# alexkeroro86/SampleNeRFRO

Measured on AMD Instinct MI355X. Metric: rays/sec (train step), higher is better.
Workload: dtype f16x3/fp32-acc

## Files before the change

### samplenerfro_amd/csrc/bkgd16.hip

```cpp
#include "mfma_ops.h"
#include "bkgd_layout.h"
#include "so3_layout.h"

namespace rnerf {

__device__ __forceinline__ void bkgd16_split2(float a, float b, uint32_t& hi, uint32_t& lo) { split2<true>(a, b, hi, lo); }
__device__ __forceinline__ void bkgd16_split8(const float (&w)[8], uint4& hi, uint4& lo) {
  uint32_t h[4], l[4];
#pragma unroll
  for (int p = 0; p < 4; ++p) bkgd16_split2(w[2 * p], w[2 * p + 1], h[p], l[p]);
  hi = make_uint4(h[0], h[1], h[2], h[3]); lo = make_uint4(l[0], l[1], l[2], l[3]);
}
template <int NS, bool FIRST, typename WF, typename LF, typename XF>
__device__ __forceinline__ void bkgd16_layer(f32x16 (&acc)[4], WF wload, LF live, bool half0, XF xop) {
  constexpr int DEPTH = 2;
  f32x2 w[DEPTH + 1][16];
  auto load = [&](int s, f32x2 (&dst)[16]) {
#pragma unroll
    for (int t = 0; t < 4; ++t)
#pragma unroll
      for (int j = 0; j < 8; ++j)
        if (live(s, j) != 0) dst[4 * t + (j >> 1)][j & 1] = wload(s, t, j);
  };
#pragma unroll
  for (int s = 0; s < DEPTH && s < NS; ++s) load(s, w[s]);
  f32x16 zero;
#pragma unroll
  for (int r = 0; r < 16; ++r) zero[r] = 0.f;
#pragma unroll
  for (int s = 0; s < NS; ++s) {
    if (s + DEPTH < NS) load(s + DEPTH, w[(s + DEPTH) % (DEPTH + 1)]);
    RNERF_PIN();
    uint4 bh, bl;
    xop(s, bh, bl);
#pragma unroll
    for (int t = 0; t < 4; ++t) {
      uint32_t hh[4], ll[4];
#pragma unroll
      for (int p = 0; p < 4; ++p) {
        const int l0 = live(s, 2 * p), l1 = live(s, 2 * p + 1);
        if (l0 == 0 && l1 == 0) { hh[p] = 0u; ll[p] = 0u; continue; }
        f32x2 q = w[s % (DEPTH + 1)][4 * t + p];
        if (l0 == 0) q[0] = 0.f;
        if (l1 == 0) q[1] = 0.f;
        q = q * 256.0f;
        if (l0 == 2) q[0] = half0 ? q[0] : 0.f;
        if (l1 == 2) q[1] = half0 ? q[1] : 0.f;
        bkgd16_split2(q[0], q[1], hh[p], ll[p]);
      }
      const uint4 ah = make_uint4(hh[0], hh[1], hh[2], hh[3]), al = make_uint4(ll[0], ll[1], ll[2], ll[3]);
      acc[t] = mfma16<true>(ah, bh, FIRST && s == 0 ? zero : acc[t]);
      acc[t] = mfma16<true>(ah, bl, acc[t]);
      acc[t] = mfma16<true>(al, bh, acc[t]);
    }
    RNERF_PIN();
  }
}
struct Bkgd16Lane {
  const float* p0;
  const float* prev;
  const float* dir;
  const float* sp;
  bool half0;
};
__device__ __forceinline__ Bkgd16Lane bkgd16_lane(const float* __restrict__ params, int m, int h) {
  return {params + m, params + m + 4 * 128 * h, params + m + 12 * 128 * h, params + m + 2 * 128 * h, h == 0};
}
template <bool BIAS>
__device__ __forceinline__ void bkgd16_prev_layer(f32x16 (&acc)[4], const f32x16 (&x)[4], const Bkgd16Lane& L, int koff, int boff) {
  bkgd16_layer<BIAS ? 9 : 8, true>(acc,
      [&](int s, int t, int j) { return s < 8 ? L.prev[koff + (16 * s + 8 * (j >> 2) + (j & 3)) * 128 + 32 * t] : L.p0[boff + 32 * t]; },
      [&](int s, int j) { return s < 8 ? 1 : (j == 0 ? 2 : 0); }, L.half0,
      [&](int s, uint4& bh, uint4& bl) {
    if (s < 8) {
      float xv[8];
#pragma unroll
      for (int j = 0; j < 8; ++j) xv[j] = x[s >> 1][8 * (s & 1) + j];
      bkgd16_split8(xv, bh, bl);
    } else {
      bh = make_uint4(L.half0 ? 0x3c00u : 0u, 0u, 0u, 0u);
      bl = make_uint4(0u, 0u, 0u, 0u);
    }
  });
}
template <bool FIRST>
__device__ __forceinline__ void bkgd16_dir_layer(f32x16 (&acc)[4], const float (&enc)[14], const Bkgd16Lane& L, int koff, int boff) {
  bkgd16_layer<2, FIRST>(acc,
      [&](int s, int t, int j) {
        const int q = 8 * s + j;
        return q < 12 ? L.dir[koff + (3 + q) * 128 + 32 * t] : (q == 12 ? L.sp[koff + 32 * t] : (q == 13 ? L.p0[koff + 128 + 32 * t] : L.p0[boff + 32 * t]));
      },
      [&](int s, int j) { const int q = 8 * s + j; return q < 13 ? 1 : (q < 15 ? 2 : 0); }, L.half0,
      [&](int s, uint4& bh, uint4& bl) {
    float xv[8];
#pragma unroll
    for (int j = 0; j < 8; ++j) xv[j] = 8 * s + j < 14 ? enc[8 * s + j] : (8 * s + j == 14 && L.half0 ? 1.0f : 0.f);
    bkgd16_split8(xv, bh, bl);
  });
}

template <bool TRAIN>
__global__ void __launch_bounds__(64) bkgd16_fwd_kernel(const float* __restrict__ params, const float* __restrict__ dirs, int dir_stride,
                                                        long long n, float pad_scale, float pad, float* __restrict__ out_rgb,
                                                        float* __restrict__ save) {
  const int lane = threadIdx.x & 63, m = lane & 31, h = lane >> 5;
  long long row = (long long)blockIdx.x * 32 + m;
  const bool ok = row < n;
  if (!ok) row = n - 1;
  const float v0 = dirs[row * dir_stride], v1 = dirs[row * dir_stride + 1], v2 = dirs[row * dir_stride + 2];
  float enc[14];
  const float phase = h ? 1.5707963705062866f : 0.0f;
#pragma unroll
  for (int q = 0; q < 12; ++q) {
    const int d = q / 3, c = q % 3;
    const float x = c == 0 ? v0 : (c == 1 ? v1 : v2);
    enc[q] = sinf(fadd(fmul(x, (float)(1 << d)), phase));
  }
  enc[12] = h ? v2 : v0;
  enc[13] = h ? 0.f : v1;
  auto save_x = [&](int k, const f32x16 (&xx)[4]) {
    if constexpr (TRAIN) {
      if (ok) {
        float* dst = save + (size_t)n * 28 + (size_t)(k - 1) * n * 128 + (size_t)row * 128;
#pragma unroll
        for (int t = 0; t < 4; ++t)
#pragma unroll
          for (int g = 0; g < 4; ++g)
            *(float4*)(dst + 32 * t + 8 * g + 4 * h) = make_float4(xx[t][4 * g], xx[t][4 * g + 1], xx[t][4 * g + 2], xx[t][4 * g + 3]);
      }
    }
  };
  if constexpr (TRAIN) {
    if (ok) {
#pragma unroll
      for (int q = 0; q < 14; ++q) { const int f = h ? dir_feature(q, 1) : dir_feature(q, 0); if (f >= 0) save[(size_t)row * 28 + f] = enc[q]; }
      if (h == 1) save[(size_t)row * 28 + 27] = 0.f;
    }
  }
  constexpr float INV = 1.0f / 256.0f;
  f32x16 acc[4], x[4];
  auto relu_to_x = [&]() {
#pragma unroll
    for (int t = 0; t < 4; ++t)
#pragma unroll
      for (int r = 0; r < 16; ++r) { const float y = acc[t][r] * INV; x[t][r] = y < 0.f ? 0.f : y; }
  };
  const Bkgd16Lane L = bkgd16_lane(params, m, h);
  bkgd16_dir_layer<true>(acc, enc, L, bkgd_koff(0), bkgd_boff(0));
  relu_to_x();
  save_x(1, x);
  bkgd16_prev_layer<true>(acc, x, L, bkgd_koff(1), bkgd_boff(1));
  relu_to_x();
  save_x(2, x);
  bkgd16_prev_layer<true>(acc, x, L, bkgd_koff(2), bkgd_boff(2));
  relu_to_x();
  save_x(3, x);
  bkgd16_prev_layer<false>(acc, x, L, bkgd_koff(3), 0);
  bkgd16_dir_layer<false>(acc, enc, L, bkgd_koff(3) + 128 * 128, bkgd_boff(3));
  relu_to_x();
  if constexpr (TRAIN) save_x(4, x);
  float o[3] = {0.f, 0.f, 0.f};
  const float* __restrict__ k4 = params + bkgd_koff(4);
#pragma unroll
  for (int t = 0; t < 4; ++t)
#pragma unroll
    for (int r = 0; r < 16; ++r) {
      const float v = x[t][r];
      const int f = 32 * t + (r & 3) + 8 * (r >> 2) + 4 * h;
      o[0] = fmaf(v, k4[f * 3 + 0], o[0]); o[1] = fmaf(v, k4[f * 3 + 1], o[1]); o[2] = fmaf(v, k4[f * 3 + 2], o[2]);
    }
#pragma unroll
  for (int c = 0; c < 3; ++c) {
    o[c] = o[c] + __shfl_xor(o[c], 32) + params[bkgd_boff(4) + c];
    o[c] = fsub(fmul(fdiv(1.0f, fadd(1.0f, expf(-o[c]))), pad_scale), pad);
  }
  if (ok && h == 0) {
    out_rgb[3 * row] = o[0]; out_rgb[3 * row + 1] = o[1]; out_rgb[3 * row + 2] = o[2];
    if constexpr (TRAIN) { float* so = save + (size_t)n * (28 + 4 * 128) + (size_t)row * 3; so[0] = o[0]; so[1] = o[1]; so[2] = o[2]; }
  }
}

static int launch_bkgd16_fwd(bool train, const float* params, const float* dirs, int dir_stride, long long n, float pad_scale, float pad, float* out_rgb,
                             float* save, hipStream_t st) {
  const dim3 grid((unsigned)((n + 31) / 32));
  if (train) hipLaunchKernelGGL(bkgd16_fwd_kernel<true>, grid, dim3(64), 0, st, params, dirs, dir_stride, n, pad_scale, pad, out_rgb, save);
  else hipLaunchKernelGGL(bkgd16_fwd_kernel<false>, grid, dim3(64), 0, st, params, dirs, dir_stride, n, pad_scale, pad, out_rgb, save);
  RNERF_CHECK_LAUNCH();
  return RNERF_OK;
}

template <bool FIRST>
__device__ __forceinline__ void so3_16_enc_layer(f32x16 (&acc)[4], const float (&enc)[30], const float* __restrict__ pe, const Bkgd16Lane& L, int koff, int boff) {
  bkgd16_layer<4, FIRST>(acc,
      [&](int s, int t, int j) { const int p = 8 * s + j; return p < 30 ? pe[koff + 2 * p * 128 + 32 * t] : L.p0[boff + 32 * t]; },
      [&](int s, int j) { const int p = 8 * s + j; return p < 30 ? 1 : (p == 30 ? 2 : 0); }, L.half0,
      [&](int s, uint4& bh, uint4& bl) {
    float xv[8];
#pragma unroll
    for (int j = 0; j < 8; ++j) { const int p = 8 * s + j; xv[j] = p < 30 ? enc[p < 30 ? p : 0] : ((p == 30 && L.half0) ? 1.0f : 0.f); }
    bkgd16_split8(xv, bh, bl);
  });
}

__global__ void __launch_bounds__(64) so3_16_fwd_train_kernel(const float* __restrict__ params, So3Window win, const float4* __restrict__ pts, long long n,
                                                              float* __restrict__ save) {
  const int lane = threadIdx.x & 63, m = lane & 31, h = lane >> 5;
  long long row = (long long)blockIdx.x * 32 + m;
  const bool ok = row < n;
  if (!ok) row = n - 1;
  const float4 pt = pts[row];
  float enc[30];
  so3_encode(pt.x, pt.y, pt.z, win, h, enc);
  if (ok) {
#pragma unroll
    for (int p = 0; p < 30; ++p) save[(size_t)row * 60 + 2 * p + h] = enc[p];
  }
  auto save_x = [&](int k, const f32x16 (&xx)[4]) {
    so3_store_mask(save, n, row, k, xx, h, ok);
    if (ok) {
      float* dst = save + (size_t)n * 60 + (size_t)(k - 1) * n * 128 + (size_t)row * 128;
#pragma unroll
      for (int t = 0; t < 4; ++t)
#pragma unroll
        for (int g = 0; g < 4; ++g)
          *(float4*)(dst + 32 * t + 8 * g + 4 * h) = make_float4(xx[t][4 * g], xx[t][4 * g + 1], xx[t][4 * g + 2], xx[t][4 * g + 3]);
    }
  };
  constexpr float INV = 1.0f / 256.0f;
  f32x16 acc[4], x[4];
  auto relu_to_x = [&]() {
#pragma unroll
    for (int t = 0; t < 4; ++t)
#pragma unroll
      for (int r = 0; r < 16; ++r) { const float y = acc[t][r] * INV; x[t][r] = y < 0.f ? 0.f : y; }
  };
  const Bkgd16Lane L = bkgd16_lane(params, m, h);
  const float* __restrict__ pe = params + m + 128 * h;
  so3_16_enc_layer<true>(acc, enc, pe, L, so3_koff(0), so3_boff(0));
  relu_to_x();
  save_x(1, x);
  bkgd16_prev_layer<true>(acc, x, L, so3_koff(1), so3_boff(1));
  relu_to_x();
  save_x(2, x);
  bkgd16_prev_layer<true>(acc, x, L, so3_koff(2), so3_boff(2));
  relu_to_x();
  save_x(3, x);
  bkgd16_prev_layer<false>(acc, x, L, so3_koff(3), 0);
  so3_16_enc_layer<false>(acc, enc, pe, L, so3_koff(3) + 128 * 128, so3_boff(3));
  relu_to_x();
  save_x(4, x);
  float o[3] = {0.f, 0.f, 0.f};
  const float* __restrict__ k4 = params + so3_koff(4);
#pragma unroll
  for (int t = 0; t < 4; ++t)
#pragma unroll
    for (int r = 0; r < 16; ++r) {
      const int f = 32 * t + (r & 3) + 8 * (r >> 2) + 4 * h;
      o[0] = fmaf(x[t][r], k4[f * 3 + 0], o[0]); o[1] = fmaf(x[t][r], k4[f * 3 + 1], o[1]); o[2] = fmaf(x[t][r], k4[f * 3 + 2], o[2]);
    }
#pragma unroll
  for (int c = 0; c < 3; ++c) o[c] = o[c] + __shfl_xor(o[c], 32) + params[so3_boff(4) + c];
  if (ok && h == 0) *(float4*)(save + (size_t)n * (60 + 4 * 128) + (size_t)row * 4) = make_float4(o[0], o[1], o[2], 0.f);
}

static int launch_so3_16_fwd_train(const float* params, So3Window win, const float* pts4, long long n, float* save, hipStream_t st) {
  hipLaunchKernelGGL(so3_16_fwd_train_kernel, dim3((unsigned)((n + 31) / 32)), dim3(64), 0, st, params, win, (const float4*)pts4, n, save);
  RNERF_CHECK_LAUNCH();
  return RNERF_OK;
}

}

using namespace rnerf;

extern "C" int rnerf_bkgd_forward(const float* params, const float* dirs, int32_t dir_stride, int64_t n, double rgb_padding,
                                  float* out_rgb, void* stream) {
  RNERF_CHECK_ARG(params && dirs && out_rgb, "rnerf_bkgd_forward: null pointer");
  RNERF_CHECK_ARG(dir_stride >= 3, "rnerf_bkgd_forward: dir_stride must be >= 3");
  RNERF_CHECK_ARG(n >= 1, "rnerf_bkgd_forward: n must be >= 1");
  return launch_bkgd16_fwd(false, params, dirs, dir_stride, (long long)n, (float)(1 + 2 * rgb_padding), (float)rgb_padding, out_rgb, nullptr, (hipStream_t)stream);
}

extern "C" int rnerf_bkgd_forward_train(const float* params, const float* dirs, int32_t dir_stride, int64_t n, double rgb_padding,
                                        float* out_rgb, void* save, void* stream) {
  RNERF_CHECK_ARG(params && dirs && out_rgb && save, "rnerf_bkgd_forward_train: null pointer");
  RNERF_CHECK_ARG(dir_stride >= 3 && n >= 1, "rnerf_bkgd_forward_train: need dir_stride >= 3 and n >= 1");
  return launch_bkgd16_fwd(true, params, dirs, dir_stride, (long long)n, (float)(1 + 2 * rgb_padding), (float)rgb_padding, out_rgb, (float*)save, (hipStream_t)stream);
}

extern "C" int rnerf_so3_forward_train(const float* so3_params, const float* window10, const float* pts4, int64_t n, void* save, void* stream) {
  RNERF_CHECK_ARG(so3_params && window10 && pts4 && save, "rnerf_so3_forward_train: null pointer");
  RNERF_CHECK_ARG(n >= 1, "rnerf_so3_forward_train: n must be >= 1");
  So3Window w;
  for (int i = 0; i < 10; ++i) w.w[i] = window10[i];
  return launch_so3_16_fwd_train(so3_params, w, pts4, (long long)n, (float*)save, (hipStream_t)stream);
}
```

### samplenerfro_amd/csrc/mlp.hip

```cpp
#include "common.h"
#include "nerfmlp_layout.h"
#include "mfma_ops.h"

#include <stdlib.h>
#include <type_traits>
#include <vector>
#include <stdio.h>

namespace rnerf {


#define GLOBAL_AS __attribute__((address_space(1)))
#define LDS_AS __attribute__((address_space(3)))

struct MfmaLayer { int dense, ks, nt, kind; };
__host__ __device__ constexpr MfmaLayer mfma_layer(int l) {
  constexpr MfmaLayer t[10] = {{0, 4, 8, 0},  {1, 16, 8, 1}, {2, 16, 8, 1}, {3, 16, 8, 1}, {4, 16, 8, 1},
                               {5, 20, 8, 2}, {6, 16, 8, 1}, {7, 16, 8, 1}, {9, 16, 8, 1}, {10, 18, 4, 3}};
  return t[l];
}
__host__ __device__ constexpr int layer_blocks_before(int l) {
  int o = 0;
  for (int i = 0; i < l; ++i) o += mfma_layer(i).ks * mfma_layer(i).nt;
  return o;
// ... 1397 lines not shown
    const int t = b / NP, part = b % NP;
    int slot0, slot1;
    const uint4* base;
    WgTrDma d;
    if (t < KT) {
      x_slots(sg, t, slot0, slot1);
      base = saved + (part ? sv_lo0(R) : 0);
      d.tstride = (unsigned)(SAVE_SLOTS * 64 * sizeof(uint4));
    } else {
      d_slots(sg, t - KT, slot0, slot1);
      base = dy + (part ? dy_plane_uint4(R, 1) : 0);
      d.tstride = (unsigned)(DY_SLOTS * 64 * sizeof(uint4));
    }
    static_assert(sv_addr(1, 0, 0, 0) == dy_addr(1, 0, 0, 0) && sv_addr(0, 0, 1, 1) == dy_addr(0, 0, 1, 1), "one lane-offset formula for both tensors");
    d.sbase = (const char*)(base + sv_addr(__builtin_amdgcn_readfirstlane(slot0), 0, 0, 0));
    d.voff = (unsigned)((sv_addr(a ? __builtin_amdgcn_readfirstlane(slot1 - slot0) : 0, 0, r, h)) * sizeof(uint4));
    d.hstride = 0;
    return d;
  }
  static __device__ __forceinline__ const char* step_src(const WgTrDma& d, size_t t32, int sc) {
    return d.sbase + t32 * d.tstride + (sc & 1) * (32 * sizeof(uint4));
  }
  template <int KT, int NT> struct Frags {
    const char* ring;
    __device__ __forceinline__ Frags(const char* ring0, int lane) : ring(ring0 + wgtr_lane_off(lane)) {}
    __device__ __forceinline__ void read_a(int t, const half8& sc8, half8& h, half8& l) const {
      const char* p = ring + t * NP * 1024;
      h = tr_read8(p) * sc8;
      if constexpr (LO) l = tr_read8(p + 1024) * sc8;
    }
    __device__ __forceinline__ void read_b(int nt, half8& h, half8& l) const {
      const char* p = ring + (KT + nt) * NP * 1024;
      h = tr_read8(p);
      if constexpr (LO) l = tr_read8(p + 1024);
    }
  };
};

__device__ __forceinline__ int2v tr_read8b(const char* p) {
  typedef __attribute__((address_space(3))) int2v lds_int2;
  return __builtin_amdgcn_ds_read_tr8_b64_v2i32((lds_int2*)p);
}
struct Lo8Planes {
  static constexpr bool LO = true;
  static constexpr int NPLANES = 2;
  static constexpr int NBUF = 4;
  static constexpr int nblk(int KT, int NT) { return KT + NT + (KT + 1) / 2 + (NT + 1) / 2; }
  static constexpr int lds_bytes() { return NBUF * wgtr_step_bytes(nblk(10, 8)); }
  template <int KT, int NT>
  static __device__ __forceinline__ WgTrDma dma(int b, int lane, const uint4* __restrict__ saved, const uint4* __restrict__ dy, long long R, const WgTrSegs& sg) {
    constexpr int NHI = KT + NT, NLX = (KT + 1) / 2;
    WgTrDma d;
    if (b < NHI) {
      const int r = lane >> 2, a = (lane >> 1) & 1, h = lane & 1;
      int s0, s1;
      const bool is_x = b < KT;
      if (is_x) x_slots(sg, b, s0, s1); else d_slots(sg, b - KT, s0, s1);
      d.sbase = (const char*)((is_x ? saved : dy) + sv_addr(__builtin_amdgcn_readfirstlane(s0), 0, 0, 0));
      d.voff = (unsigned)((sv_addr(a ? __builtin_amdgcn_readfirstlane(s1 - s0) : 0, 0, r, h)) * sizeof(uint4));
      d.tstride = (unsigned)((is_x ? SAVE_SLOTS : DY_SLOTS) * 64 * sizeof(uint4));
      d.hstride = (unsigned)(32 * sizeof(uint4));
      return d;
    }
    const int lb = b - NHI;
    const bool is_x = lb < NLX;
    const int t0 = 2 * (is_x ? lb : lb - NLX) + (lane >> 5);
    const int r = (lane & 31) >> 1, a = lane & 1;
    int s0, s1;
    if (is_x) x_slots(sg, t0 < KT ? t0 : KT - 1, s0, s1); else d_slots(sg, t0 < NT ? t0 : NT - 1, s0, s1);
    d.sbase = is_x ? (const char*)(saved + sv_lo0(R)) : (const char*)(dy + dy_plane_uint4(R, 1));
    d.voff = (unsigned)(((a ? s1 : s0) * 32 + r) * 16);
    d.tstride = (unsigned)((is_x ? SAVE_SLOTS : DY_SLOTS) * 32 * 16);
    d.hstride = 16u * 16u;
    return d;
  }
  static __device__ __forceinline__ const char* step_src(const WgTrDma& d, size_t t32, int sc) {
    return d.sbase + t32 * d.tstride + (sc & 1) * d.hstride;
  }
  template <int KT, int NT> struct Frags {
    static constexpr int LOX = (KT + NT) * 1024, LOD = LOX + (KT + 1) / 2 * 1024;
    const char *ring, *ring8;
    __device__ __forceinline__ Frags(const char* ring0, int lane)
        : ring(ring0 + wgtr_lane_off(lane)), ring8(ring0 + (unsigned)((8 * (lane >> 5) + ((lane & 15) >> 1)) * 32 + ((lane >> 4) & 1) * 16 + (lane & 1) * 8)) {}
    __device__ __forceinline__ void read_a(int t, const half8& sc8, half8& h, half8& l) const {
      h = tr_read8(ring + t * 1024) * sc8;
      l = lo8_decode(tr_read8b(ring8 + LOX + t * 512), LO8_SCALE_X) * sc8;
    }
    __device__ __forceinline__ void read_b(int nt, half8& h, half8& l) const {
      h = tr_read8(ring + (KT + nt) * 1024);
      l = lo8_decode(tr_read8b(ring8 + LOD + nt * 512), LO8_SCALE_D);
    }
  };
};

template <class Planes, int KT, int NT>
__device__ __forceinline__ void wgrad_body_tr(const uint4* __restrict__ saved, const uint4* __restrict__ dy, long long R, float* __restrict__ pg,
                                               float* __restrict__ pbias, const WgTrSegs sg, int g, int G, char* smem) {
  using SH = WgTrShape<KT, NT>;
  constexpr int TK = SH::TK, TN = SH::TN;
  constexpr int NBLK = Planes::nblk(KT, NT), NDMA = (NBLK + 7) / 8, STEP_BYTES = wgtr_step_bytes(NBLK);
  constexpr int WGTR_NBUF = Planes::NBUF, AHEAD = WGTR_NBUF - 1;
  static_assert((WGTR_NBUF & (WGTR_NBUF - 1)) == 0, "ring slots are addressed with a mask");
  const int tid = threadIdx.x, lane = tid & 63;
  const int wave = __builtin_amdgcn_readfirstlane(tid >> 6);
  const int wk = wave / SH::WN, wn = wave % SH::WN;
  const bool active = wave < SH::WK * SH::WN;
  const float* __restrict__ rs = (const float*)(dy + dy_plane_uint4(R, Planes::NPLANES));
  const float mref = rs[R];
  const float inv_mref = mref > 0.f ? 1.0f / mref : 0.f;
  WgTrDma blk[NDMA];
  unsigned lds_blk[NDMA];
#pragma unroll
  for (int i = 0; i < NDMA; ++i) {
    int b = wave + 8 * i;
    b = b < NBLK ? b : NBLK - 1;
    blk[i] = Planes::template dma<KT, NT>(b, lane, saved, dy, R, sg);
    lds_blk[i] = (unsigned)b * 1024u;
  }
  const float* rs_src = rs + 4 * (lane & 3);
  const long long n_t32 = R / 32;
  const int my_tiles = g < n_t32 ? (int)((n_t32 - 1 - g) / G) + 1 : 0;
  const int n_steps = 2 * my_tiles;
  auto issue = [&](int s) {
    const int sc = s < n_steps ? s : n_steps - 1;
    const size_t t32 = (size_t)g + (size_t)(sc >> 1) * G;
    const unsigned ring = (unsigned)(s & (WGTR_NBUF - 1)) * STEP_BYTES;
#pragma unroll
    for (int i = 0; i < NDMA; ++i)
      glds16_nt_s(Planes::step_src(blk[i], t32, sc), blk[i].voff, __builtin_amdgcn_readfirstlane(ring + lds_blk[i]));
    if (wave == 0) glds16_nt((const char*)(rs_src + t32 * 32 + (sc & 1) * 16), __builtin_amdgcn_readfirstlane(ring + NBLK * 1024u));
  };
  const f32x16 zero = {0, 0, 0, 0, 0, 0, 0, 0, 0, 0, 0, 0, 0, 0, 0, 0};
  f32x16 acc[TK][TN], acce = zero;
  float accb = 0.f;
#pragma unroll
  for (int i = 0; i < TK; ++i)
#pragma unroll
    for (int j = 0; j < TN; ++j) acc[i][j] = zero;
  if (n_steps > 0) {
#pragma unroll
    for (int s = 0; s < AHEAD; ++s) issue(s);
    const int kh = lane >> 5;
    for (int s = 0; s < n_steps; ++s) {
      if (wave == 0) wait_vmcnt<(AHEAD - 1) * (NDMA + 1)>(); else
      wait_vmcnt<(AHEAD - 1) * NDMA>();
      __syncthreads();
      issue(s + AHEAD);
      if (active) {
        const char* ring0 = smem + (s & (WGTR_NBUF - 1)) * STEP_BYTES;
        const typename Planes::template Frags<KT, NT> frags(ring0, lane);
        const float4 s0 = *(const float4*)(ring0 + NBLK * 1024 + kh * 32), s1 = *(const float4*)(ring0 + NBLK * 1024 + kh * 32 + 16);
        const half8 sc8 = {(_Float16)(s0.x * inv_mref), (_Float16)(s0.y * inv_mref), (_Float16)(s0.z * inv_mref), (_Float16)(s0.w * inv_mref),
                           (_Float16)(s1.x * inv_mref), (_Float16)(s1.y * inv_mref), (_Float16)(s1.z * inv_mref), (_Float16)(s1.w * inv_mref)};
        half8 beh, bel;
        if constexpr (SH::EXTRA) frags.read_b(NT - 1, beh, bel);
        static_assert(SH::WK >= TN, "bias owners");
        auto read_a = [&](int i, half8& h, half8& l) { frags.read_a(wk * TK + i, sc8, h, l); };
        auto read_b = [&](int j, half8& h, half8& l) { frags.read_b(wn * TN + j, h, l); };
        auto dot8 = [&](const half8& x, float c) -> float {
#pragma unroll
          for (int k = 0; k < 4; ++k) c = __builtin_amdgcn_fdot2(half2v{sc8[2 * k], sc8[2 * k + 1]}, half2v{x[2 * k], x[2 * k + 1]}, c, false);
          return c;
        };
        auto bias_row = [&](int j, const half8& h, const half8& l) {
          if (wk == j) {
            accb = dot8(h, accb);
            if constexpr (Planes::LO) accb = dot8(l, accb);
          }
        };
        half8 ae_h, ae_l;
        if constexpr (TK > TN) {
          half8 bh[TN], bl[TN];
#pragma unroll
          for (int j = 0; j < TN; ++j) read_b(j, bh[j], bl[j]);
          half8 an_h, an_l;
          read_a(0, an_h, an_l);
#pragma unroll
          for (int i = 0; i < TK; ++i) {
            const half8 ah = an_h, al = an_l;
            if (i + 1 < TK) read_a(i + 1, an_h, an_l);
#pragma unroll
            for (int j = 0; j < TN; ++j) acc[i][j] = mfma_h8(ah, bh[j], acc[i][j]);
            if constexpr (Planes::LO) {
#pragma unroll
              for (int j = 0; j < TN; ++j) acc[i][j] = mfma_h8(ah, bl[j], acc[i][j]);
#pragma unroll
              for (int j = 0; j < TN; ++j) acc[i][j] = mfma_h8(al, bh[j], acc[i][j]);
            }
          }
#pragma unroll
          for (int j = 0; j < TN; ++j) bias_row(j, bh[j], bl[j]);
        } else {
          constexpr int NCH = WGTR_NCH < TN ? WGTR_NCH : TN;
          static_assert(TN % NCH == 0, "n-tile chunks");
          half8 ah[TK], al[TK];
#pragma unroll
          for (int i = 0; i < TK; ++i) read_a(i, ah[i], al[i]);
#pragma unroll
          for (int c = 0; c < TN / NCH; ++c) {
            half8 bh[NCH], bl[NCH];
#pragma unroll
            for (int jj = 0; jj < NCH; ++jj) read_b(c * NCH + jj, bh[jj], bl[jj]);
#pragma unroll
            for (int i = 0; i < TK; ++i)
#pragma unroll
              for (int jj = 0; jj < NCH; ++jj) acc[i][c * NCH + jj] = mfma_h8(ah[i], bh[jj], acc[i][c * NCH + jj]);
            if constexpr (Planes::LO) {
#pragma unroll
              for (int i = 0; i < TK; ++i)
#pragma unroll
                for (int jj = 0; jj < NCH; ++jj) acc[i][c * NCH + jj] = mfma_h8(ah[i], bl[jj], acc[i][c * NCH + jj]);
#pragma unroll
              for (int i = 0; i < TK; ++i)
#pragma unroll
                for (int jj = 0; jj < NCH; ++jj) acc[i][c * NCH + jj] = mfma_h8(al[i], bh[jj], acc[i][c * NCH + jj]);
            }
#pragma unroll
            for (int jj = 0; jj < NCH; ++jj) bias_row(c * NCH + jj, bh[jj], bl[jj]);
          }
          if constexpr (SH::EXTRA) { ae_h = wn ? ah[1] : ah[0]; if constexpr (Planes::LO) ae_l = wn ? al[1] : al[0]; }
        }
        if constexpr (SH::EXTRA) {
          static_assert(!SH::EXTRA || TK <= TN, "the extra tile reads the resident A fragments");
          acce = mfma_h8(ae_h, beh, acce);
          if constexpr (Planes::LO) {
            acce = mfma_h8(ae_h, bel, acce);
            acce = mfma_h8(ae_l, beh, acce);
          }
        }
      }
    }
    wait_vmcnt<0>();
  }
  constexpr size_t ldn = (size_t)NT * 32;
  const int m = lane & 31, h = lane >> 5;
  if (active) {
#pragma unroll
    for (int i = 0; i < TK; ++i)
#pragma unroll
      for (int j = 0; j < TN; ++j)
#pragma unroll
        for (int r = 0; r < 16; ++r) {
          const int row = (r & 3) + 8 * (r >> 2) + 4 * h;
          pg[(size_t)((wk * TK + i) * 32 + row) * ldn + (wn * TN + j) * 32 + m] = acc[i][j][r];
        }
    if constexpr (SH::EXTRA) {
#pragma unroll
      for (int r = 0; r < 16; ++r) {
        const int row = (r & 3) + 8 * (r >> 2) + 4 * h;
        pg[(size_t)((wk * TK + wn) * 32 + row) * ldn + (NT - 1) * 32 + m] = acce[r];
      }
    }
    const float bsum = accb + __shfl_xor(accb, 32);
    if (wk < TN && h == 0) pbias[(wn * TN + wk) * 32 + m] = bsum;
  }
}

constexpr int WGRAD_VGPRS = 112;
template <class Planes>
__global__ void __launch_bounds__(512) __attribute__((amdgpu_num_vgpr(WGRAD_VGPRS)))
nerfmlp_wgrad_tr_kernel(const uint4* __restrict__ saved, const uint4* __restrict__ dy, long long R, float* __restrict__ workspace, const WgradTable tab,
                        long long* __restrict__ trace) {
  extern __shared__ __attribute__((aligned(16))) char smem[];
  if (trace && threadIdx.x == 0) trace[2 * blockIdx.x] = (long long)__builtin_amdgcn_s_memrealtime();
  int j = 0;
  while ((int)blockIdx.x >= tab.wg0[j + 1]) ++j;
  const WgradJob job = tab.job[j];
  const int g = blockIdx.x - tab.wg0[j], G = tab.wg0[j + 1] - tab.wg0[j];
  const int KT = job.KT, NT = job.NT;
  float* pg = workspace + tab.poff[j] + (size_t)g * (size_t)KT * 32 * NT * 32;
  float* pb = workspace + tab.pboff[j] + (size_t)g * NT * 32;
  const WgTrSegs sg = {tab.qx[j], job.KTa, tab.qx2[j], tab.qd[j], job.NTa, tab.KSd[j], tab.qd2[j], tab.KSd2[j]};
#define RNERF_WGRAD_CASE(KT_, NT_)                                                                                                  \
  if (KT == (KT_) && NT == (NT_)) {                                                                                                 \
    wgrad_body_tr<Planes, KT_, NT_>(saved, dy, R, pg, pb, sg, g, G, smem);                                                          \
    if (trace && threadIdx.x == 0) trace[2 * blockIdx.x + 1] = (long long)__builtin_amdgcn_s_memrealtime();                         \
    return;                                                                                                                         \
  }
  RNERF_WGRAD_CASE(8, 8) RNERF_WGRAD_CASE(2, 8) RNERF_WGRAD_CASE(10, 8) RNERF_WGRAD_CASE(8, 9) RNERF_WGRAD_CASE(9, 4) RNERF_WGRAD_CASE(4, 1)
#undef RNERF_WGRAD_CASE
  __builtin_trap();
}

template <bool X_F16>
__global__ void __launch_bounds__(512)
nerfmlp_wgrad_kernel(const uint4* __restrict__ saved, const uint4* __restrict__ dy, long long R, long long total_rows, int n_chunks,
                      float* __restrict__ workspace, const WgradTable tab) {
  extern __shared__ __attribute__((aligned(16))) char smem[];
  int j = 0;
  while ((int)blockIdx.x >= tab.wg0[j + 1]) ++j;
  const int qx = tab.qx[j], KSx = tab.KSx[j], qd = tab.qd[j], KSd = tab.KSd[j];
  const int g = blockIdx.x - tab.wg0[j], G = tab.wg0[j + 1] - tab.wg0[j];
  const int KT = KSx >> 1, NT = (KSd + 1) >> 1;
  float* pg = workspace + tab.poff[j] + (size_t)g * (size_t)KT * 32 * NT * 32;
  float* pb = workspace + tab.pboff[j] + (size_t)g * NT * 32;
#define RNERF_WGRAD_CASE(KT_, KSD_)                                                                                                 \
  if (KSx == 2 * (KT_) && KSd == (KSD_)) { wgrad_body<X_F16, KT_, KSD_>(saved, dy, R, total_rows, n_chunks, pg, pb, qx, qd, g, G, smem); return; }
  RNERF_WGRAD_CASE(8, 16) RNERF_WGRAD_CASE(2, 16) RNERF_WGRAD_CASE(8, 1) RNERF_WGRAD_CASE(8, 8) RNERF_WGRAD_CASE(1, 8) RNERF_WGRAD_CASE(4, 1)
#undef RNERF_WGRAD_CASE
  __builtin_trap();
}

__global__ void __launch_bounds__(256) wgrad_reduce_kernel(const float* __restrict__ workspace, const WgradTable tab, float* __restrict__ grads,
                                                           const float* __restrict__ out_scale) {
  const float osc = out_scale ? *out_scale : 1.0f;
  const int jb = blockIdx.y;
  const WgradJob job = tab.job[jb];
  const int n_wg = tab.wg0[jb + 1] - tab.wg0[jb];
  const float* __restrict__ partial = workspace + tab.poff[jb];
  const float* __restrict__ partial_bias = workspace + tab.pboff[jb];
  const int ldn = job.NT * 32, rows = job.KT * 32;
  const int e = blockIdx.x * blockDim.x + threadIdx.x;
  auto out_feature = [&](int J, int& dense) -> int {
    int nt = J >> 5;
    const int c = J & 31, a = c >> 4, hh = (c >> 3) & 1, j = c & 7;
    const bool segb = nt >= job.NTa;
    const int dkind = segb ? job.dkind2 : job.dkind;
    dense = segb ? job.dense2 : job.dense;
    if (segb) nt -= job.NTa;
    if (dkind == 0) { const int n = prev_feature(2 * nt + a, hh, j); return n < nerf_dense(dense).out ? n : -1; }
    if (a != 0 || hh != 0 || nt != 0) return -1;
    if (dkind == 1) return j == 0 ? 0 : -1;
    return (j >= 1 && j <= 3) ? j - 1 : -1;
  };
  auto sum_over = [&](const float* __restrict__ p, size_t stride) -> float {
    float s0 = 0.f, s1 = 0.f, s2 = 0.f, s3 = 0.f;
    int g = 0;
    for (; g + 4 <= n_wg; g += 4) { s0 += p[(size_t)g * stride]; s1 += p[(size_t)(g + 1) * stride]; s2 += p[(size_t)(g + 2) * stride]; s3 += p[(size_t)(g + 3) * stride]; }
    for (; g < n_wg; ++g) s0 += p[(size_t)g * stride];
    return (s0 + s1) + (s2 + s3);
  };
  if (e < rows * ldn) {
    const int I = e / ldn, J = e % ldn;
    int kt = I >> 5;
    const int c = I & 31, a = c >> 4, hh = (c >> 3) & 1, j = c & 7;
    const bool segb = kt >= job.KTa;
    const int xkind = segb ? job.xkind2 : job.xkind, row_off = segb ? job.row_off2 : job.row_off;
    if (segb) kt -= job.KTa;
    const int s = 2 * kt + a;
    int fin = xkind == 1 ? prev_feature(s, hh, j) : (xkind == 0 ? pe_feature(8 * s + j, hh) : view_feature(8 * s + j, hh));
    int dense;
    const int fout = out_feature(J, dense);
    if (fin >= 0 && fout >= 0) {
      fin += row_off;
      if (fin < nerf_dense(dense).in) grads[nerf_koff(dense) + fin * nerf_dense(dense).out + fout] = sum_over(partial + e, (size_t)rows * ldn) * osc;
    }
  }
  if (job.write_bias && e < ldn) {
    int dense;
    const int fout = out_feature(e, dense);
    if (fout >= 0 && (e >> 5) < job.NTa) grads[nerf_boff(dense) + fout] = sum_over(partial_bias + e, (size_t)ldn) * osc;
    if (job.bias_sigma && e == 0) grads[nerf_boff(8)] = sum_over(partial_bias, (size_t)ldn) * osc;
  }
}

template <int NP>
__global__ void __launch_bounds__(64) nerfmlp_input_grad_kernel(const float* __restrict__ params, const uint4* __restrict__ dy, long long R,
                                                                const float4* __restrict__ rows_pd, const float4* __restrict__ rows_dr,
                                                                const int* __restrict__ node_of_sample, int B, long long total_rows,
                                                                float4* __restrict__ d_pos, float4* __restrict__ d_dir) {
  const int lane = threadIdx.x & 63, m = lane & 31, h = lane >> 5;
  long long row = (long long)blockIdx.x * 32 + m;
  const bool ok = row < total_rows;
  if (!ok) row = total_rows - 1;
  const f32x16 zero = {0, 0, 0, 0, 0, 0, 0, 0, 0, 0, 0, 0, 0, 0, 0, 0};
  f32x16 dpe[2] = {zero, zero}, dve = zero;
  auto slot_vals = [&](int q, float (&vals)[8]) {
    const uint4 hi = dy[dy_addr(q, row >> 5, (int)(row & 31), h)];
    const uint32_t hw[4] = {hi.x, hi.y, hi.z, hi.w};
#pragma unroll
    for (int p = 0; p < 4; ++p) unpack2<true>(hw[p], vals[2 * p], vals[2 * p + 1]);
    if constexpr (NP == 2) {
      const uint4 lo = dy[dy_plane_uint4(R, 1) + dy_addr(q, row >> 5, (int)(row & 31), h)];
      const uint32_t lw[4] = {lo.x, lo.y, lo.z, lo.w};
#pragma unroll
      for (int p = 0; p < 4; ++p) { float a, b; unpack2<true>(lw[p], a, b); vals[2 * p] += a; vals[2 * p + 1] += b; }
    }
    if constexpr (NP == 3) {
      const uint2 lo = ((const uint2*)(dy + dy_plane_uint4(R, 1)))[dy_addr(q, row >> 5, (int)(row & 31), h)];
      const half8 lv = lo8_decode(int2v{(int)lo.x, (int)lo.y}, LO8_SCALE_D);
#pragma unroll
      for (int j = 0; j < 8; ++j) vals[j] += (float)lv[j];
    }
  };
  auto gemm_T = [&](const float* __restrict__ kern, int out_dim, int row0, int fin, int slot0, int nslots, f32x16* acc, int ntile) {
    const float* __restrict__ kr[2];
    bool live[2];
#pragma unroll
    for (int t2 = 0; t2 < 2; ++t2) {
      const int f = 32 * t2 + m;
      live[t2] = f < fin;
      kr[t2] = kern + (size_t)(row0 + (f < fin ? f : fin - 1)) * out_dim + 4 * h;
    }
    float4 wc[2][2], wn[2][2];
    float vc[8], vn[8];
    auto fetch = [&](int s, float4 (&w)[2][2], float (&vals)[8]) {
#pragma unroll
      for (int t2 = 0; t2 < 2; ++t2)
        if (t2 < ntile) { w[t2][0] = *(const float4*)(kr[t2] + 16 * s); w[t2][1] = *(const float4*)(kr[t2] + 16 * s + 8); }
      slot_vals(slot0 + s, vals);
    };
    fetch(0, wc, vc);
#pragma unroll 1
    for (int s = 0; s < nslots; ++s) {
      if (s + 1 < nslots) fetch(s + 1, wn, vn);
      RNERF_PIN();
#pragma unroll
      for (int j = 0; j < 8; ++j) {
#pragma unroll
        for (int t2 = 0; t2 < 2; ++t2) {
          if (t2 < ntile) {
            const float4 q = wc[t2][j >> 2];
            const float w = (j & 3) == 0 ? q.x : ((j & 3) == 1 ? q.y : ((j & 3) == 2 ? q.z : q.w));
            acc[t2] = __builtin_amdgcn_mfma_f32_32x32x2f32(live[t2] ? w : 0.f, vc[j], acc[t2], 0, 0, 0);
          }
        }
      }
      RNERF_PIN();
#pragma unroll
      for (int t2 = 0; t2 < 2; ++t2) { wc[t2][0] = wn[t2][0]; wc[t2][1] = wn[t2][1]; }
#pragma unroll
      for (int j = 0; j < 8; ++j) vc[j] = vn[j];
    }
  };
  gemm_T(params + nerf_koff(0), 256, 0, 63, 0, 16, dpe, 2);
  gemm_T(params + nerf_koff(5), 256, 256, 63, 16 * 5, 16, dpe, 2);
  gemm_T(params + nerf_koff(10), 128, 256, 27, DY_L9, 8, &dve, 1);
  size_t rec = (size_t)row;
  if (node_of_sample) { const long long sidx = row / B; rec = (size_t)node_of_sample[sidx] * B + (size_t)(row - sidx * B); }
  const float4 pd = rows_pd[rec], dr = rows_dr[rec];
  const float pc[3] = {pd.x, pd.y, pd.z}, dcv[3] = {dr.x, dr.y, dr.z};
  const float HALF_PI = 1.5707963705062866f;
  float gp3[3] = {0.f, 0.f, 0.f}, gd3[3] = {0.f, 0.f, 0.f};
#pragma unroll
  for (int t2 = 0; t2 < 2; ++t2)
#pragma unroll
    for (int r = 0; r < 16; ++r) {
      const int f = 32 * t2 + (r & 3) + 8 * (r >> 2) + 4 * h;
      if (f < 3) gp3[f] += dpe[t2][r];
      else if (f < 63) {
        const int q = (f - 3) % 30, is_cos = (f - 3) / 30, d = q / 3, c = q % 3;
        const float xb = fmul(pc[c], (float)(1 << d));
        gp3[c] = fmaf(dpe[t2][r], (float)(1 << d) * pe_cos(is_cos ? fadd(xb, HALF_PI) : xb), gp3[c]);
      }
    }
#pragma unroll
  for (int r = 0; r < 16; ++r) {
    const int f = (r & 3) + 8 * (r >> 2) + 4 * h;
    if (f < 3) gd3[f] += dve[r];
    else if (f < 27) {
      const int q = (f - 3) % 12, is_cos = (f - 3) / 12, d = q / 3, c = q % 3;
      const float xb = fmul(dcv[c], (float)(1 << d));
      gd3[c] = fmaf(dve[r], (float)(1 << d) * pe_cos(is_cos ? fadd(xb, HALF_PI) : xb), gd3[c]);
    }
  }
  const float* __restrict__ rs = (const float*)(dy + dy_plane_uint4(R, NP == 3 ? 2 : NP));
  const float sc = rs[row];
#pragma unroll
  for (int c = 0; c < 3; ++c) { gp3[c] = (gp3[c] + __shfl_xor(gp3[c], 32)) * sc; gd3[c] = (gd3[c] + __shfl_xor(gd3[c], 32)) * sc; }
  if (ok && h == 0) { d_pos[row] = make_float4(gp3[0], gp3[1], gp3[2], 0.f); d_dir[row] = make_float4(gd3[0], gd3[1], gd3[2], 0.f); }
}

}

namespace rnerf {
int launch_fwd_f32(const void* packed, const float* rows_pd, const float* rows_dr, const int32_t* node_of_sample, int32_t B, long long total_rows,
                   float* out_raw, hipStream_t st);
}

using namespace rnerf;

constexpr size_t kF8Fallback = (Prec<RNERF_PREC_F16F8>::PACKED_BYTES + 255) & ~(size_t)255;

constexpr size_t kX3Bytes = (Prec<RNERF_PREC_F16X3>::PACKED_BYTES + 255) & ~(size_t)255;
constexpr size_t kSafeBytes = Prec<RNERF_PREC_BF16X3>::PACKED_BYTES;
constexpr size_t kF16Bytes = (Prec<RNERF_PREC_F16>::PACKED_BYTES + 255) & ~(size_t)255;
static size_t safe_stream_offset(int precision) {
  switch (precision) {
    case RNERF_PREC_F16X3:
    case RNERF_PREC_F16X2: return kX3Bytes;
    case RNERF_PREC_F16F8: return kF8Fallback + kX3Bytes;
    case RNERF_PREC_F16: return kF16Bytes;
    default: return 0;
  }
}

#define RNERF_TRY_(expr) do { int rc_ = (expr); if (rc_ != RNERF_OK) return rc_; } while (0)

static bool prec_ok(int p) {
  return p == RNERF_PREC_F32 || p == RNERF_PREC_F16X3 || p == RNERF_PREC_BF16X3 || p == RNERF_PREC_F16 || p == RNERF_PREC_BF16 || p == RNERF_PREC_F16X2 || p == RNERF_PREC_F16F8;
}

extern "C" size_t rnerf_nerfmlp_packed_bytes(int precision) {
  switch (precision) {
    case RNERF_PREC_F32: return (size_t)RNERF_NERFMLP_PARAMS * sizeof(float);
    case RNERF_PREC_F16X3:
    case RNERF_PREC_F16X2: return kX3Bytes + kSafeBytes;
    case RNERF_PREC_F16F8: return kF8Fallback + kX3Bytes + kSafeBytes;
    case RNERF_PREC_BF16X3: return Prec<RNERF_PREC_BF16X3>::PACKED_BYTES;
    case RNERF_PREC_F16: return kF16Bytes + kSafeBytes;
    case RNERF_PREC_BF16: return Prec<RNERF_PREC_BF16>::PACKED_BYTES;
    default: set_error("rnerf_nerfmlp_packed_bytes: unsupported precision %d", precision); return 0;
  }
}

namespace rnerf {
void* nerfmlp_dgrad_scale_ref(int backward, void* dy, int64_t rows);
static int pack_flag_regions(int precision, void* packed, void** out) {
  auto at = [&](size_t off) { return (void*)((char*)packed + off + AUX_FLAG * sizeof(float)); };
  switch (precision) {
    case RNERF_PREC_F16X3:
    case RNERF_PREC_F16X2: out[0] = at(Prec<RNERF_PREC_F16X3>::STREAM_BYTES); return 1;
    case RNERF_PREC_F16F8: out[0] = at(Prec<RNERF_PREC_F16F8>::STREAM_BYTES); out[1] = at(kF8Fallback + Prec<RNERF_PREC_F16X3>::STREAM_BYTES); return 2;
    case RNERF_PREC_F16: out[0] = at(Prec<RNERF_PREC_F16>::STREAM_BYTES); return 1;
    default: return 0;
  }
}
struct FlagRegions { float4* p[12]; };
__global__ void __launch_bounds__(64) zero_flags_kernel(FlagRegions r, int n) {
  if ((int)threadIdx.x < n) *r.p[threadIdx.x] = make_float4(0.f, 0.f, 0.f, 0.f);
}
int nerfmlp_step_zero(int precision, void* const* packed, int count, int backward, void* const* dy, const int64_t* dy_rows, int dy_count, hipStream_t st) {
  FlagRegions r;
  int n = 0;
  for (int i = 0; i < count && i < 2; ++i) { void* o[2]; const int k = pack_flag_regions(precision, packed[i], o); for (int q = 0; q < k; ++q) r.p[n++] = (float4*)o[q]; }
  for (int i = 0; i < dy_count && i < 4; ++i) { void* f = nerfmlp_dgrad_scale_ref(backward, dy[i], dy_rows[i]); if (f) r.p[n++] = (float4*)f; }
  if (n == 0) return RNERF_OK;
  hipLaunchKernelGGL(zero_flags_kernel, dim3(1), dim3(64), 0, st, r, n);
  RNERF_CHECK_LAUNCH();
  return RNERF_OK;
}

int nerfmlp_pack_impl(const float* params, int precision, void* packed, bool zero_flags, hipStream_t st, bool with_safe) {
  const int threads = kTotalBlocks * 64, block = 256, grid = (threads + block - 1) / block;
  if (zero_flags) {
    void* o[2];
    const int k = pack_flag_regions(precision, packed, o);
    for (int q = 0; q < k; ++q) RNERF_CHECK_HIP(hipMemsetAsync(o[q], 0, 4 * sizeof(float), st));
  }
  switch (precision) {
    case RNERF_PREC_F32:
      RNERF_CHECK_HIP(hipMemcpyAsync(packed, params, (size_t)RNERF_NERFMLP_PARAMS * sizeof(float), hipMemcpyDeviceToDevice, st));
      return RNERF_OK;
    case RNERF_PREC_F16X3:
    case RNERF_PREC_F16X2: hipLaunchKernelGGL(nerfmlp_pack_kernel<RNERF_PREC_F16X3>, dim3(grid), dim3(block), 0, st, params, (char*)packed); break;
    case RNERF_PREC_F16F8:
      hipLaunchKernelGGL(nerfmlp_pack_kernel<RNERF_PREC_F16F8>, dim3(grid), dim3(block), 0, st, params, (char*)packed);
      hipLaunchKernelGGL(nerfmlp_pack_kernel<RNERF_PREC_F16X3>, dim3(grid), dim3(block), 0, st, params, (char*)packed + kF8Fallback);
      break;
    case RNERF_PREC_F16: hipLaunchKernelGGL(nerfmlp_pack_kernel<RNERF_PREC_F16>, dim3(grid), dim3(block), 0, st, params, (char*)packed); break;
    case RNERF_PREC_BF16X3: hipLaunchKernelGGL(nerfmlp_pack_kernel<RNERF_PREC_BF16X3>, dim3(grid), dim3(block), 0, st, params, (char*)packed); break;
    default: hipLaunchKernelGGL(nerfmlp_pack_kernel<RNERF_PREC_BF16>, dim3(grid), dim3(block), 0, st, params, (char*)packed); break;
  }
  if (with_safe && safe_stream_offset(precision) != 0)
    hipLaunchKernelGGL(nerfmlp_pack_kernel<RNERF_PREC_BF16X3>, dim3(grid), dim3(block), 0, st, params, (char*)packed + safe_stream_offset(precision));
  RNERF_CHECK_LAUNCH();
  return RNERF_OK;
}
}

extern "C" int rnerf_nerfmlp_pack(const float* params, int precision, void* packed, void* stream) {
  RNERF_CHECK_ARG(params && packed, "rnerf_nerfmlp_pack: null pointer");
  RNERF_CHECK_ARG(prec_ok(precision), "rnerf_nerfmlp_pack: unsupported precision %d", precision);
  RNERF_CHECK_ARG(((uintptr_t)packed & 15) == 0, "rnerf_nerfmlp_pack: packed must be 16-byte aligned");
  return nerfmlp_pack_impl(params, precision, packed, true, (hipStream_t)stream, true);
}

constexpr size_t SAVE_QUEUE_BYTES = 8192;
static size_t save_payload_bytes(long long padded, bool with_lo) {
  return (size_t)(SAVE_TOTAL + (with_lo ? SAVE_SLOTS : 0)) * (size_t)padded * 2 * sizeof(uint4);
}

template <int PREC, int MODE = 0, int TRAIN = 0>
static int launch_fwd_mode(const void* packed, const float* rows_pd, const float* rows_dr, const int32_t* node_of_sample, int32_t B,
                           long long total_rows, float* out_raw, hipStream_t st, void* save = nullptr, int max_wg = 0, const float* gate = nullptr,
                           int gate_skip_if = 0) {
  using PP = Prec<PREC>;
  const int n_tiles = (int)((total_rows + 255) / 256);
  int dev = 0, cus = 0;
  RNERF_CHECK_HIP(hipGetDevice(&dev));
  RNERF_CHECK_HIP(hipDeviceGetAttribute(&cus, hipDeviceAttributeMultiprocessorCount, dev));
  const int lim = (max_wg > 0 && max_wg < cus) ? max_wg : cus;
  if constexpr (MODE == 0 && (PREC == RNERF_PREC_F16X3 || PREC == RNERF_PREC_F16F8)) {
    static const bool half_ok = [] { const char* e = RNERF_ENV("RNERF_FWD_HALF_TILES"); return !(e && e[0] == '0'); }();
    if (half_ok && 2 * n_tiles <= lim) {
      const size_t lds1 = 2 * (size_t)PP::SLAB;
      static DeviceOnce attr1_set;
      if (attr1_set.need()) {
        RNERF_CHECK_HIP(hipFuncSetAttribute((const void*)nerfmlp_fwd_kernel<PREC, 0, TRAIN, true>, hipFuncAttributeMaxDynamicSharedMemorySize, (int)lds1));
        attr1_set.set();
      }
      hipLaunchKernelGGL((nerfmlp_fwd_kernel<PREC, 0, TRAIN, true>), dim3(2 * n_tiles), dim3(256), lds1, st, (const char*)packed, (const float4*)rows_pd,
                         (const float4*)rows_dr, node_of_sample, B, total_rows, 2 * n_tiles, (float4*)out_raw, (uint4*)save, (long long)n_tiles * 256,
                         (int*)nullptr, gate, gate_skip_if);
      RNERF_CHECK_LAUNCH();
      return RNERF_OK;
    }
  }
  const int grid = n_tiles < lim ? n_tiles : lim;
  const size_t lds = 2 * (size_t)PP::SLAB + 4 * 32768;
  static DeviceOnce attr_set;
  if (attr_set.need()) {
    RNERF_CHECK_HIP(hipFuncSetAttribute((const void*)nerfmlp_fwd_kernel<PREC, MODE, TRAIN>, hipFuncAttributeMaxDynamicSharedMemorySize, (int)lds));
    attr_set.set();
  }
  int* tileq = nullptr;
  if (TRAIN != 0 && grid < cus && grid < n_tiles) {
    tileq = (int*)((char*)save + save_payload_bytes((long long)n_tiles * 256, TRAIN >= 2));
    RNERF_CHECK_HIP(hipMemsetAsync(tileq, 0, sizeof(int), st));
  }
  hipLaunchKernelGGL((nerfmlp_fwd_kernel<PREC, MODE, TRAIN>), dim3(grid), dim3(256), lds, st, (const char*)packed, (const float4*)rows_pd,
                     (const float4*)rows_dr, node_of_sample, B, total_rows, n_tiles, (float4*)out_raw, (uint4*)save,
                     (long long)n_tiles * 256, tileq, gate, gate_skip_if);
  RNERF_CHECK_LAUNCH();
  return RNERF_OK;
}

template <int PREC>
static int launch_fwd(const void* packed, const float* rows_pd, const float* rows_dr, const int32_t* node_of_sample, int32_t B,
                      long long total_rows, float* out_raw, hipStream_t st, int max_wg, const float* gate = nullptr, int gate_skip_if = 0) {
  return launch_fwd_mode<PREC>(packed, rows_pd, rows_dr, node_of_sample, B, total_rows, out_raw, st, nullptr, max_wg, gate, gate_skip_if);
}

extern "C" int rnerf_nerfmlp_forward(const void* packed, int precision, const float* rows_pd, const float* rows_dr,
                                     const int32_t* node_of_sample, int32_t S, int32_t B, float* out_raw, int32_t max_workgroups,
                                     void* stream) {
  RNERF_CHECK_ARG(packed && rows_pd && rows_dr && out_raw, "rnerf_nerfmlp_forward: null pointer");
  RNERF_CHECK_ARG(max_workgroups >= 0, "rnerf_nerfmlp_forward: max_workgroups must be >= 0");
  RNERF_CHECK_ARG(prec_ok(precision), "rnerf_nerfmlp_forward: unsupported precision %d", precision);
  RNERF_CHECK_ARG(S >= 1 && B >= 1, "rnerf_nerfmlp_forward: need S >= 1 and B >= 1");
  RNERF_CHECK_ARG((((uintptr_t)packed | (uintptr_t)rows_pd | (uintptr_t)rows_dr | (uintptr_t)out_raw) & 15) == 0,
                  "rnerf_nerfmlp_forward: buffers must be 16-byte aligned");
  const long long total = (long long)S * B;
  hipStream_t st = (hipStream_t)stream;
  switch (precision) {
    case RNERF_PREC_F32: return launch_fwd_f32(packed, rows_pd, rows_dr, node_of_sample, B, total, out_raw, st);
    case RNERF_PREC_F16X3:
      RNERF_TRY_(launch_fwd<RNERF_PREC_F16X3>(packed, rows_pd, rows_dr, node_of_sample, B, total, out_raw, st, max_workgroups));
      return launch_fwd_mode<RNERF_PREC_BF16X3, 512>((const char*)packed + safe_stream_offset(precision), rows_pd, rows_dr, node_of_sample, B, total, out_raw, st, nullptr, max_workgroups);
    case RNERF_PREC_F16X2:
      RNERF_TRY_(launch_fwd<RNERF_PREC_F16X2>(packed, rows_pd, rows_dr, node_of_sample, B, total, out_raw, st, max_workgroups));
      return launch_fwd_mode<RNERF_PREC_BF16X3, 512>((const char*)packed + safe_stream_offset(precision), rows_pd, rows_dr, node_of_sample, B, total, out_raw, st, nullptr, max_workgroups);
    case RNERF_PREC_F16F8: {
      const float* flag = (const float*)((const char*)packed + Prec<RNERF_PREC_F16F8>::STREAM_BYTES) + AUX_FLAG;
      RNERF_TRY_(launch_fwd<RNERF_PREC_F16F8>(packed, rows_pd, rows_dr, node_of_sample, B, total, out_raw, st, max_workgroups, flag, 1));
      RNERF_TRY_(launch_fwd<RNERF_PREC_F16X3>((const char*)packed + kF8Fallback, rows_pd, rows_dr, node_of_sample, B, total, out_raw, st, max_workgroups, flag, 0));
      return launch_fwd_mode<RNERF_PREC_BF16X3, 512>((const char*)packed + safe_stream_offset(precision), rows_pd, rows_dr, node_of_sample, B, total, out_raw, st, nullptr, max_workgroups);
    }
    case RNERF_PREC_BF16X3: return launch_fwd<RNERF_PREC_BF16X3>(packed, rows_pd, rows_dr, node_of_sample, B, total, out_raw, st, max_workgroups);
    case RNERF_PREC_F16:
      RNERF_TRY_(launch_fwd<RNERF_PREC_F16>(packed, rows_pd, rows_dr, node_of_sample, B, total, out_raw, st, max_workgroups));
      return launch_fwd_mode<RNERF_PREC_BF16X3, 512>((const char*)packed + safe_stream_offset(precision), rows_pd, rows_dr, node_of_sample, B, total, out_raw, st, nullptr, max_workgroups);
    default: return launch_fwd<RNERF_PREC_BF16>(packed, rows_pd, rows_dr, node_of_sample, B, total, out_raw, st, max_workgroups);
  }
}

static bool bwd_ok(int b) { return b == RNERF_BWD_BF16 || b == RNERF_BWD_F16 || b == RNERF_BWD_F16X2 || b == RNERF_BWD_F16X3_LO8; }
static bool bwd_two_planes(int b) { return b == RNERF_BWD_F16X2 || b == RNERF_BWD_F16X3_LO8; }
static bool train_combo_ok(int precision, int backward) {
  return precision == RNERF_PREC_F16X3 || (precision == RNERF_PREC_F16 && !bwd_two_planes(backward)) ||
         (precision == RNERF_PREC_BF16X3 && backward == RNERF_BWD_BF16);
}
static size_t train_stream_bytes(int precision) {
  return precision == RNERF_PREC_F16 ? Prec<RNERF_PREC_F16>::STREAM_BYTES : (precision == RNERF_PREC_BF16X3 ? Prec<RNERF_PREC_BF16X3>::STREAM_BYTES : Prec<RNERF_PREC_F16X3>::STREAM_BYTES);
}

extern "C" size_t rnerf_nerfmlp_save_bytes(int64_t rows, int backward) {
  const int64_t padded = (rows + 255) / 256 * 256;
  return save_payload_bytes(padded, bwd_two_planes(backward)) + SAVE_QUEUE_BYTES;
}

extern "C" int rnerf_nerfmlp_forward_train(const void* packed, int precision, const float* rows_pd, const float* rows_dr,
                                           const int32_t* node_of_sample, int32_t S, int32_t B, float* out_raw, void* save,
                                           int backward, int32_t max_workgroups, void* stream) {
  RNERF_CHECK_ARG(packed && rows_pd && rows_dr && out_raw && save, "rnerf_nerfmlp_forward_train: null pointer");
  RNERF_CHECK_ARG(max_workgroups >= 0, "rnerf_nerfmlp_forward_train: max_workgroups must be >= 0");
  RNERF_CHECK_ARG(bwd_ok(backward), "rnerf_nerfmlp_forward_train: unknown backward mode %d", backward);
  RNERF_CHECK_ARG(train_combo_ok(precision, backward),
                  "rnerf_nerfmlp_forward_train: the training forward is built for precision f16x3, f16 with the single-plane backward modes, and bf16x3 with backward bf16");
  RNERF_CHECK_ARG(S >= 1 && B >= 1, "rnerf_nerfmlp_forward_train: need S >= 1 and B >= 1");
  RNERF_CHECK_ARG((((uintptr_t)packed | (uintptr_t)rows_pd | (uintptr_t)rows_dr | (uintptr_t)out_raw | (uintptr_t)save) & 15) == 0,
                  "rnerf_nerfmlp_forward_train: buffers must be 16-byte aligned");
  const long long total = (long long)S * B;
  hipStream_t st = (hipStream_t)stream;
  if (backward == RNERF_BWD_F16X2) return launch_fwd_mode<RNERF_PREC_F16X3, 0, 2>(packed, rows_pd, rows_dr, node_of_sample, B, total, out_raw, st, save, max_workgroups);
  if (backward == RNERF_BWD_F16X3_LO8) return launch_fwd_mode<RNERF_PREC_F16X3, 0, 3>(packed, rows_pd, rows_dr, node_of_sample, B, total, out_raw, st, save, max_workgroups);
  if (precision == RNERF_PREC_BF16X3) return launch_fwd_mode<RNERF_PREC_BF16X3, 0, 1>(packed, rows_pd, rows_dr, node_of_sample, B, total, out_raw, st, save, max_workgroups);
  if (precision == RNERF_PREC_F16) return launch_fwd_mode<RNERF_PREC_F16, 0, 1>(packed, rows_pd, rows_dr, node_of_sample, B, total, out_raw, st, save, max_workgroups);
  return launch_fwd_mode<RNERF_PREC_F16X3, 0, 1>(packed, rows_pd, rows_dr, node_of_sample, B, total, out_raw, st, save, max_workgroups);
}

extern "C" size_t rnerf_nerfmlp_bwd_packed_bytes(void) { return (size_t)kBwdBlocks * 2 * 1024; }
extern "C" size_t rnerf_nerfmlp_dy_bytes(int64_t rows, int backward) {
  const int64_t padded = (rows + 255) / 256 * 256;
  const int np = bwd_two_planes(backward) ? 2 : 1;
  return dy_plane_uint4(padded, np) * sizeof(uint4) + (backward == RNERF_BWD_BF16 ? 0 : ((size_t)padded + 4) * sizeof(float));
}

extern "C" int rnerf_nerfmlp_pack_bwd(const float* params, int backward, void* packed_bwd, void* stream) {
  RNERF_CHECK_ARG(params && packed_bwd, "rnerf_nerfmlp_pack_bwd: null pointer");
  RNERF_CHECK_ARG(bwd_ok(backward), "rnerf_nerfmlp_pack_bwd: unknown backward mode %d", backward);
  const int threads = kBwdBlocks * 64;
  if (backward == RNERF_BWD_BF16)
    hipLaunchKernelGGL(nerfmlp_pack_bwd_kernel<RNERF_PREC_BF16X3>, dim3((threads + 255) / 256), dim3(256), 0, (hipStream_t)stream, params, (char*)packed_bwd);
  else
    hipLaunchKernelGGL(nerfmlp_pack_bwd_kernel<RNERF_PREC_F16X3>, dim3((threads + 255) / 256), dim3(256), 0, (hipStream_t)stream, params, (char*)packed_bwd);
  RNERF_CHECK_LAUNCH();
  return RNERF_OK;
}

void* rnerf::nerfmlp_dgrad_scale_ref(int backward, void* dy, int64_t rows) {
  const long long R = (rows + 255) / 256 * 256;
  if (bwd_two_planes(backward)) return (char*)dy + dy_plane_uint4(R, Bwd<RNERF_BWD_F16X2>::NP) * sizeof(uint4) + (size_t)R * sizeof(float);
  if (backward == RNERF_BWD_F16) return (char*)dy + dy_plane_uint4(R, Bwd<RNERF_BWD_F16>::NP) * sizeof(uint4) + (size_t)R * sizeof(float);
  return nullptr;
}

template <int BWD>
static int launch_dgrad(const void* packed_bwd, const float* fwd_aux, const void* save, const float* d_raw, int64_t rows, void* dy, hipStream_t st,
                        bool zero_ref = true, bool allow_half = true) {
  using PB = Prec<Bwd<BWD>::PREC>;
  const int n_tiles = (int)((rows + 255) / 256);
  int dev = 0, cus = 0;
  RNERF_CHECK_HIP(hipGetDevice(&dev));
  RNERF_CHECK_HIP(hipDeviceGetAttribute(&cus, hipDeviceAttributeMultiprocessorCount, dev));
  const int grid = n_tiles < cus ? n_tiles : cus;
  const size_t lds = 2 * (size_t)PB::SLAB + 4 * 32768;
  static DeviceOnce attr_set;
  if (attr_set.need()) {
    RNERF_CHECK_HIP(hipFuncSetAttribute((const void*)nerfmlp_dgrad_kernel<BWD>, hipFuncAttributeMaxDynamicSharedMemorySize, (int)lds));
    attr_set.set();
  }
  const long long R = (long long)n_tiles * 256;
  if (Bwd<BWD>::F16 && zero_ref) RNERF_CHECK_HIP(hipMemsetAsync(nerfmlp_dgrad_scale_ref(BWD == kBwdF16OnePass ? RNERF_BWD_F16 : BWD, dy, rows), 0, 4 * sizeof(float), st));
  if constexpr (BWD == RNERF_BWD_F16X2 || BWD == RNERF_BWD_F16 || BWD == kBwdF16OnePass || BWD == RNERF_BWD_F16X3_LO8) {
    static const int half_lim = [] { const char* e = RNERF_ENV("RNERF_DGRAD_HALF_TILES"); return e ? atoi(e) : -1; }();
    if (allow_half && half_lim != 0 && 2 * n_tiles <= (half_lim > 1 ? half_lim : cus)) {
      const size_t lds1 = 2 * (size_t)PB::SLAB;
      static DeviceOnce attr1_set;
      if (attr1_set.need()) {
        RNERF_CHECK_HIP(hipFuncSetAttribute((const void*)nerfmlp_dgrad_kernel<BWD, true>, hipFuncAttributeMaxDynamicSharedMemorySize, (int)lds1));
        attr1_set.set();
      }
      hipLaunchKernelGGL((nerfmlp_dgrad_kernel<BWD, true>), dim3(2 * n_tiles), dim3(256), lds1, st, (const char*)packed_bwd, fwd_aux, (const uint4*)save, R,
                         (const float4*)d_raw, (long long)rows, 2 * n_tiles, (uint4*)dy);
      RNERF_CHECK_LAUNCH();
      return RNERF_OK;
    }
  }
  hipLaunchKernelGGL(nerfmlp_dgrad_kernel<BWD>, dim3(grid), dim3(256), lds, st, (const char*)packed_bwd, fwd_aux, (const uint4*)save, R,
                     (const float4*)d_raw, (long long)rows, n_tiles, (uint4*)dy);
  RNERF_CHECK_LAUNCH();
  return RNERF_OK;
}

namespace rnerf {
int nerfmlp_dgrad_impl(const void* packed_bwd, const void* packed_fwd, int fwd_precision, int backward, const void* save, const float* d_raw, int64_t rows,
                       void* dy, bool zero_ref, bool allow_half, hipStream_t st) {
  RNERF_CHECK_ARG(packed_bwd && packed_fwd && save && d_raw && dy, "rnerf_nerfmlp_dgrad: null pointer");
  RNERF_CHECK_ARG(train_combo_ok(fwd_precision, backward), "rnerf_nerfmlp_dgrad: forward precision must be f16x3 (f16 with a single-plane backward mode; bf16x3 with backward bf16)");
  RNERF_CHECK_ARG(bwd_ok(backward), "rnerf_nerfmlp_dgrad: unknown backward mode %d", backward);
  RNERF_CHECK_ARG(rows >= 1, "rnerf_nerfmlp_dgrad: rows must be >= 1");
  const float* fwd_aux = (const float*)((const char*)packed_fwd + train_stream_bytes(fwd_precision));
  if (backward == RNERF_BWD_F16X2) return launch_dgrad<RNERF_BWD_F16X2>(packed_bwd, fwd_aux, save, d_raw, rows, dy, st, zero_ref, allow_half);
  if (backward == RNERF_BWD_F16X3_LO8) return launch_dgrad<RNERF_BWD_F16X3_LO8>(packed_bwd, fwd_aux, save, d_raw, rows, dy, st, zero_ref, allow_half);
  if (backward == RNERF_BWD_F16 && fwd_precision == RNERF_PREC_F16) return launch_dgrad<kBwdF16OnePass>(packed_bwd, fwd_aux, save, d_raw, rows, dy, st, zero_ref, allow_half);
  if (backward == RNERF_BWD_F16) return launch_dgrad<RNERF_BWD_F16>(packed_bwd, fwd_aux, save, d_raw, rows, dy, st, zero_ref, allow_half);
  return launch_dgrad<RNERF_BWD_BF16>(packed_bwd, fwd_aux, save, d_raw, rows, dy, st, zero_ref, allow_half);
}
}

extern "C" int rnerf_nerfmlp_dgrad(const void* packed_bwd, const void* packed_fwd, int fwd_precision, int backward, const void* save,
                                   const float* d_raw, int64_t rows, void* dy, void* stream) {
  return nerfmlp_dgrad_impl(packed_bwd, packed_fwd, fwd_precision, backward, save, d_raw, rows, dy, true, true, (hipStream_t)stream);
}

struct WgradPlan { int qx, KSx, qd, KSd; WgradJob job; int qx2, qd2, KSd2; };
static constexpr WgradJob job1(int dense, int xkind, int row_off, int dkind, int KT, int NT, int wb, int bias_sigma = 0) {
  return WgradJob{dense, xkind, row_off, dkind, KT, NT, wb, KT, 0, 0, NT, 0, 0, bias_sigma};
}
static const WgradPlan kWgradPlan[15] = {
    {SAVE_PE, 4, 0, 16, job1(0, 0, 0, 0, 2, 8, 1), 0, 0, 0},
    {SAVE_L1 + 0, 16, 16, 16, job1(1, 1, 0, 0, 8, 8, 1), 0, 0, 0},   {SAVE_L1 + 16, 16, 32, 16, job1(2, 1, 0, 0, 8, 8, 1), 0, 0, 0},
    {SAVE_L1 + 32, 16, 48, 16, job1(3, 1, 0, 0, 8, 8, 1), 0, 0, 0},  {SAVE_L1 + 48, 16, 64, 16, job1(4, 1, 0, 0, 8, 8, 1), 0, 0, 0},
    {SAVE_L1 + 64, 16, 80, 16, job1(5, 1, 0, 0, 8, 8, 1), 0, 0, 0},  {SAVE_PE, 4, 80, 16, job1(5, 0, 256, 0, 2, 8, 0), 0, 0, 0},
    {SAVE_L1 + 80, 16, 96, 16, job1(6, 1, 0, 0, 8, 8, 1), 0, 0, 0},  {SAVE_L1 + 96, 16, 112, 16, job1(7, 1, 0, 0, 8, 8, 1), 0, 0, 0},
    {SAVE_L1 + 112, 16, 128, 16, job1(9, 1, 0, 0, 8, 8, 1), 0, 0, 0}, {SAVE_L1 + 112, 16, DY_HEADS, 1, job1(8, 1, 0, 1, 8, 1, 1), 0, 0, 0},
    {SAVE_L1 + 128, 16, DY_L9, 8, job1(10, 1, 0, 0, 8, 4, 1), 0, 0, 0}, {SAVE_VIEW, 2, DY_L9, 8, job1(10, 2, 256, 0, 1, 4, 0), 0, 0, 0},
    {SAVE_RGBIN, 8, DY_HEADS, 1, job1(11, 1, 0, 2, 4, 1, 1), 0, 0, 0},
    {0, 0, 0, 0, job1(0, 0, 0, 0, 0, 0, 0), 0, 0, 0}};
static const WgradPlan kWgradPlanTr[12] = {
    {SAVE_PE, 4, 0, 16, job1(0, 0, 0, 0, 2, 8, 1), 0, 0, 0},
    {SAVE_L1 + 0, 16, 16, 16, job1(1, 1, 0, 0, 8, 8, 1), 0, 0, 0},   {SAVE_L1 + 16, 16, 32, 16, job1(2, 1, 0, 0, 8, 8, 1), 0, 0, 0},
    {SAVE_L1 + 32, 16, 48, 16, job1(3, 1, 0, 0, 8, 8, 1), 0, 0, 0},  {SAVE_L1 + 48, 16, 64, 16, job1(4, 1, 0, 0, 8, 8, 1), 0, 0, 0},
    {SAVE_L1 + 64, 20, 80, 16, WgradJob{5, 1, 0, 0, 10, 8, 1,  8,  0,  256,  8, 0, 0, 0}, SAVE_PE, 0, 0},
    {SAVE_L1 + 80, 16, 96, 16, job1(6, 1, 0, 0, 8, 8, 1), 0, 0, 0},  {SAVE_L1 + 96, 16, 112, 16, job1(7, 1, 0, 0, 8, 8, 1), 0, 0, 0},
    {SAVE_L1 + 112, 16, 128, 16, WgradJob{9, 1, 0, 0, 8, 9, 1, 8, 0, 0,  8,  8,  1, 0}, 0, DY_HEADS, 1},
    {SAVE_L1 + 128, 18, DY_L9, 8, WgradJob{10, 1, 0, 0, 9, 4, 1,  8,  2,  256, 4, 0, 0, 0}, SAVE_VIEW, 0, 0},
    {SAVE_RGBIN, 8, DY_HEADS, 1, job1(11, 1, 0, 2, 4, 1, 1,  1), 0, 0, 0},
    {0, 0, 0, 0, job1(0, 0, 0, 0, 0, 0, 0), 0, 0, 0}};

static size_t build_wgrad_table(int cus, WgradTable& t, bool legacy, int mult = 0) {
  const WgradPlan* plan = legacy ? kWgradPlan : kWgradPlanTr;
  int n = 0;
  double cost[16], total = 0;
  for (; plan[n].KSx != 0; ++n) {
    const WgradJob& jb = plan[n].job;
    cost[n] = legacy ? 2.0 * jb.KT * jb.NT + 2 * (jb.KT + jb.NT) + 16 : jb.KT + jb.NT + 1;
    total += cost[n];
  }
  t.n = n;
  const int budget = (mult > 0 ? mult : (legacy ? 4 : 2)) * cus;
  size_t off = 0;
  int wg = 0;
  for (int i = 0; i < n; ++i) {
    const WgradPlan& p = plan[i];
    int share = (int)(budget * cost[i] / total + 0.5);
    if (share < 8) share = 8;
    t.qx[i] = p.qx; t.KSx[i] = p.KSx; t.qd[i] = p.qd; t.KSd[i] = p.KSd; t.job[i] = p.job;
    t.qx2[i] = p.qx2; t.qd2[i] = p.qd2; t.KSd2[i] = p.KSd2;
    t.wg0[i] = wg; wg += share;
    t.poff[i] = (long long)off; off += (size_t)share * p.job.KT * 32 * p.job.NT * 32;
    t.pboff[i] = (long long)off; off += (size_t)share * p.job.NT * 32;
  }
  t.wg0[n] = wg;
  return off;
}

static int device_cus() {
  int dev = 0, cus = 256;
  if (hipGetDevice(&dev) == hipSuccess) hipDeviceGetAttribute(&cus, hipDeviceAttributeMultiprocessorCount, dev);
  return cus;
}

constexpr long long kWgradSmallRows = 24576;
struct WgradTables { WgradTable legacy, tr, tr_small; size_t partial_floats; int max_wgs; };
static const WgradTables& wgrad_tables() {
  static const WgradTables tables = [] {
    WgradTables w;
    const size_t a = build_wgrad_table(device_cus(), w.legacy, true), b = build_wgrad_table(device_cus(), w.tr, false);
    const size_t s = build_wgrad_table(device_cus(), w.tr_small, false, 1);
    w.partial_floats = a > b ? a : b;
    if (s > w.partial_floats) w.partial_floats = s;
    w.max_wgs = w.legacy.wg0[w.legacy.n] > w.tr.wg0[w.tr.n] ? w.legacy.wg0[w.legacy.n] : w.tr.wg0[w.tr.n];
    if (w.tr_small.wg0[w.tr_small.n] > w.max_wgs) w.max_wgs = w.tr_small.wg0[w.tr_small.n];
    return w;
  }();
  return tables;
}

extern "C" size_t rnerf_nerfmlp_wgrad_workspace_bytes(void) {
  const WgradTables& w = wgrad_tables();
  return w.partial_floats * sizeof(float) + (size_t)w.max_wgs * 2 * sizeof(long long);
}

template <class Planes> struct WgradTrHost {
  static hipError_t allow_lds() {
    return hipFuncSetAttribute((const void*)nerfmlp_wgrad_tr_kernel<Planes>, hipFuncAttributeMaxDynamicSharedMemorySize, Planes::lds_bytes());
  }
  static const float* launch(const WgradTable& tab, hipStream_t st, const void* save, const void* dy, long long R, void* workspace, long long* trace) {
    hipLaunchKernelGGL(nerfmlp_wgrad_tr_kernel<Planes>, dim3(tab.wg0[tab.n]), dim3(512), Planes::lds_bytes(), st, (const uint4*)save, (const uint4*)dy, R,
                       (float*)workspace, tab, trace);
    return (const float*)((const uint4*)dy + dy_plane_uint4(R, Planes::NPLANES)) + R;
  }
};

extern "C" int rnerf_nerfmlp_wgrad(int fwd_precision, int backward, const void* save, const void* dy, int64_t rows, float* grads, void* workspace,
                                   void* stream) {
  RNERF_CHECK_ARG(save && dy && grads && workspace, "rnerf_nerfmlp_wgrad: null pointer");
  RNERF_CHECK_ARG(train_combo_ok(fwd_precision, backward), "rnerf_nerfmlp_wgrad: forward precision must be f16x3 (f16 with a single-plane backward mode; bf16x3 with backward bf16)");
  RNERF_CHECK_ARG(bwd_ok(backward), "rnerf_nerfmlp_wgrad: unknown backward mode %d", backward);
  RNERF_CHECK_ARG(rows >= 1, "rnerf_nerfmlp_wgrad: rows must be >= 1");
  const WgradTables& w = wgrad_tables();
  static DeviceOnce ready;
  if (ready.need()) {
    RNERF_CHECK_HIP(hipFuncSetAttribute((const void*)nerfmlp_wgrad_kernel<true>, hipFuncAttributeMaxDynamicSharedMemorySize, 131072));
    RNERF_CHECK_HIP(hipFuncSetAttribute((const void*)nerfmlp_wgrad_kernel<false>, hipFuncAttributeMaxDynamicSharedMemorySize, 131072));
    RNERF_CHECK_HIP(WgradTrHost<F16Planes<1>>::allow_lds());
    RNERF_CHECK_HIP(WgradTrHost<F16Planes<2>>::allow_lds());
    RNERF_CHECK_HIP(WgradTrHost<Lo8Planes>::allow_lds());
    ready.set();
  }
  const long long R = (rows + 255) / 256 * 256;
  hipStream_t st = (hipStream_t)stream;
  const float* out_scale = nullptr;
  static const bool tracing = RNERF_ENV("RNERF_WGRAD_TRACE") != nullptr;
  long long* trace = tracing ? (long long*)((char*)workspace + w.partial_floats * sizeof(float)) : nullptr;
  const WgradTable& tab = backward == RNERF_BWD_BF16 ? w.legacy : (rows <= kWgradSmallRows ? w.tr_small : w.tr);
  if (backward == RNERF_BWD_BF16) {
    const int n_chunks = (int)((rows + 127) / 128);
    if (fwd_precision == RNERF_PREC_BF16X3)
      hipLaunchKernelGGL(nerfmlp_wgrad_kernel<false>, dim3(tab.wg0[tab.n]), dim3(512), 131072, st, (const uint4*)save, (const uint4*)dy, R,
                         (long long)rows, n_chunks, (float*)workspace, tab);
    else
      hipLaunchKernelGGL(nerfmlp_wgrad_kernel<true>, dim3(tab.wg0[tab.n]), dim3(512), 131072, st, (const uint4*)save, (const uint4*)dy, R,
                         (long long)rows, n_chunks, (float*)workspace, tab);
  } else if (backward == RNERF_BWD_F16) {
    out_scale = WgradTrHost<F16Planes<1>>::launch(tab, st, save, dy, R, workspace, trace);
  } else if (backward == RNERF_BWD_F16X3_LO8) {
    out_scale = WgradTrHost<Lo8Planes>::launch(tab, st, save, dy, R, workspace, trace);
  } else {
    out_scale = WgradTrHost<F16Planes<2>>::launch(tab, st, save, dy, R, workspace, trace);
  }
  int max_elems = 0;
  for (int j = 0; j < tab.n; ++j) max_elems = tab.job[j].KT * tab.job[j].NT * 1024 > max_elems ? tab.job[j].KT * tab.job[j].NT * 1024 : max_elems;
  hipLaunchKernelGGL(wgrad_reduce_kernel, dim3((max_elems + 255) / 256, tab.n), dim3(256), 0, st, (const float*)workspace, tab, grads, out_scale);
  RNERF_CHECK_LAUNCH();
  if (trace && backward != RNERF_BWD_BF16) {
    const int n_wg = tab.wg0[tab.n];
    std::vector<long long> h(2 * (size_t)n_wg);
    RNERF_CHECK_HIP(hipStreamSynchronize(st));
    RNERF_CHECK_HIP(hipMemcpy(h.data(), trace, h.size() * sizeof(long long), hipMemcpyDeviceToHost));
    long long t0 = h[0];
    for (int i = 0; i < n_wg; ++i) t0 = h[2 * i] < t0 ? h[2 * i] : t0;
    for (int j = 0; j < tab.n; ++j) {
      long long a = -1, b = 0; double busy = 0;
      for (int i = tab.wg0[j]; i < tab.wg0[j + 1]; ++i) { a = (a < 0 || h[2 * i] < a) ? h[2 * i] : a; b = h[2 * i + 1] > b ? h[2 * i + 1] : b; busy += (double)(h[2 * i + 1] - h[2 * i]); }
      fprintf(stderr, "[wgrad trace] job %2d (KT %d NT %d) wgs %4d  first start %9lld  last end %9lld  mean wg ticks (100 MHz) %7.0f\n", j, tab.job[j].KT, tab.job[j].NT,
              tab.wg0[j + 1] - tab.wg0[j], a - t0, b - t0, busy / (tab.wg0[j + 1] - tab.wg0[j]));
    }
  }
  return RNERF_OK;
}

extern "C" int rnerf_nerfmlp_input_grad(const float* params, int backward, const void* dy, const float* rows_pd, const float* rows_dr,
                                        const int32_t* node_of_sample, int32_t S, int32_t B, float* d_pos4, float* d_dir4, void* stream) {
  RNERF_CHECK_ARG(params && dy && rows_pd && rows_dr && d_pos4 && d_dir4, "rnerf_nerfmlp_input_grad: null pointer");
  RNERF_CHECK_ARG(backward == RNERF_BWD_F16 || backward == RNERF_BWD_F16X2 || backward == RNERF_BWD_F16X3_LO8, "rnerf_nerfmlp_input_grad: needs the row-normalised f16 backward modes");
  RNERF_CHECK_ARG(S >= 1 && B >= 1, "rnerf_nerfmlp_input_grad: need S >= 1 and B >= 1");
  const long long rows = (long long)S * B;
  const long long R = (rows + 255) / 256 * 256;
  const unsigned grid = (unsigned)((rows + 31) / 32);
  hipStream_t st = (hipStream_t)stream;
  if (backward == RNERF_BWD_F16X3_LO8)
    hipLaunchKernelGGL(nerfmlp_input_grad_kernel<3>, dim3(grid), dim3(64), 0, st, params, (const uint4*)dy, R, (const float4*)rows_pd, (const float4*)rows_dr,
                       node_of_sample, B, rows, (float4*)d_pos4, (float4*)d_dir4);
  else if (backward == RNERF_BWD_F16X2)
    hipLaunchKernelGGL(nerfmlp_input_grad_kernel<2>, dim3(grid), dim3(64), 0, st, params, (const uint4*)dy, R, (const float4*)rows_pd, (const float4*)rows_dr,
                       node_of_sample, B, rows, (float4*)d_pos4, (float4*)d_dir4);
  else
    hipLaunchKernelGGL(nerfmlp_input_grad_kernel<1>, dim3(grid), dim3(64), 0, st, params, (const uint4*)dy, R, (const float4*)rows_pd, (const float4*)rows_dr,
                       node_of_sample, B, rows, (float4*)d_pos4, (float4*)d_dir4);
  RNERF_CHECK_LAUNCH();
  return RNERF_OK;
}
```

### samplenerfro_amd/csrc/pipeline.hip

```cpp
#include "common.h"

#include <math.h>
#include <mutex>
#include <utility>
#include <vector>

namespace rnerf {
static int current_device_cus() {
  static int cache[64] = {0};
  int dev = 0;
  if (hipGetDevice(&dev) != hipSuccess || dev < 0 || dev >= 64) return 256;
  if (cache[dev] == 0) {
    int cus = 0;
    cache[dev] = (hipDeviceGetAttribute(&cus, hipDeviceAttributeMultiprocessorCount, dev) == hipSuccess && cus > 0) ? cus : 256;
  }
  return cache[dev];
}

namespace {
constexpr size_t kPoolCap = 32;
struct EventPool { std::vector<hipEvent_t> free_[64]; };
thread_local EventPool tl_pool;
inline hipError_t pool_get(hipEvent_t* e) {
  int dev = 0;
// ... 181 lines not shown
  const double t = (double)count + 1.0;
  double lr;
  if (c.use_override) {
    lr = c.lr_override;
  } else {
    double delay = 1.0;
    if (c.lr_delay_steps > 0) {
      const double x = fmin(fmax((double)count / c.lr_delay_steps, 0.0), 1.0);
      delay = c.lr_delay_mult + (1.0 - c.lr_delay_mult) * sin(0.5 * 3.141592653589793 * x);
    }
    const double start = fmin(fmax((double)count, 0.0), 1.0);
    const double tt = fmin(fmax(fmax((double)count, 0.0) / c.max_steps, 0.0), 1.0);
    lr = start * delay * exp(log(c.lr_init) * (1.0 - tt) + log(c.lr_final) * tt);
  }
  const double bad = red[0];
  out[0] = (float)(-lr / (1.0 - pow(c.b1, t)));
  out[1] = (c.skip_nonfinite && bad > 0.0) ? -1.0f : (float)(1.0 / (1.0 - pow(c.b2, t)));
  float mult = 1.0f;
  if (c.max_norm > 0) {
    const float norm = sqrtf((float)sumsq);
    mult = fminf((float)c.max_norm / (1e-7f + norm), 1.0f);
  }
  out[2] = mult;
  out[3] = (float)bad;
}
__global__ void __launch_bounds__(256) adam_scalars_kernel(AdamSched c, int* __restrict__ step, const float* __restrict__ partial, int n_partial,
                                                           const float* __restrict__ bad_partial, float* __restrict__ scal) {
  __shared__ double red[256];
  const int count = *step;
  adam_scalars_block(c, count, partial, n_partial, bad_partial, red, scal);
  if (threadIdx.x == 0) *step = count + 1;
}
__global__ void __launch_bounds__(256) adam_apply_kernel(float* __restrict__ theta, float* __restrict__ mu, float* __restrict__ nu,
                                                         const float* __restrict__ g, long long n, float b1, float b2, float eps,
                                                         float* __restrict__ scal, int count_bad) {
  const float a = scal[0], c2 = scal[1], mult = scal[2];
  if (c2 < 0.f) return;
  int bad = 0;
  for (long long i = (long long)blockIdx.x * blockDim.x + threadIdx.x; i < n; i += (long long)gridDim.x * blockDim.x) {
    const float gi = g[i] * mult;
    bad += !(fabsf(gi) <= 3.402823466e38f);
    const float m = mu[i] * b1 + gi * (1.0f - b1);
    const float v = nu[i] * b2 + (gi * gi) * (1.0f - b2);
    mu[i] = m; nu[i] = v;
    theta[i] = theta[i] + a * (m / (sqrtf(v * c2) + eps));
  }
  if (count_bad && __builtin_amdgcn_ballot_w64(bad != 0) != 0) {
    for (int o = 32; o > 0; o >>= 1) bad += __shfl_down(bad, o);
    if ((threadIdx.x & 63) == 0 && bad) atomicAdd(&scal[3], (float)bad);
  }
}

__global__ void __launch_bounds__(256) adam_apply_fused_kernel(AdamSched c, const int* __restrict__ step, const float* __restrict__ partial,
                                                               int n_partial, const float* __restrict__ bad_partial, float* __restrict__ theta,
                                                               float* __restrict__ mu, float* __restrict__ nu, const float* __restrict__ g,
                                                               long long n, float b1, float b2, float eps, float* __restrict__ scal,
                                                               float* __restrict__ count_out) {
  __shared__ double red[256];
  __shared__ float sc[4];
  adam_scalars_block(c, *step - 1, partial, n_partial, bad_partial, red, sc);
  __syncthreads();
  const float a = sc[0], c2 = sc[1], mult = sc[2];
  if (blockIdx.x == 0 && threadIdx.x == 0) {
    scal[0] = a; scal[1] = c2; scal[2] = mult; scal[3] = sc[3];
    if (count_out) *count_out = sc[3];
  }
  if (c2 < 0.f) return;
  for (long long i = (long long)blockIdx.x * blockDim.x + threadIdx.x; i < n; i += (long long)gridDim.x * blockDim.x) {
    const float gi = g[i] * mult;
    const float m = mu[i] * b1 + gi * (1.0f - b1);
    const float v = nu[i] * b2 + (gi * gi) * (1.0f - b2);
    mu[i] = m; nu[i] = v;
    theta[i] = theta[i] + a * (m / (sqrtf(v * c2) + eps));
  }
}

struct Carver {
  char* base; size_t off;
  explicit Carver(void* b) : base((char*)b), off(0) {}
  template <typename T> T* take(size_t count) {
    off = (off + 255) & ~(size_t)255;
    T* p = (T*)(base ? base + off : nullptr);
    off += count * sizeof(T);
    return p;
  }
  void* bytes(size_t n) { return (void*)take<char>(n); }
};

struct FwdBuffers {
  float *path_pd, *path_dr, *bk_dirs, *bkgd, *raw_c, *weights, *u, *rows_pd, *rows_dr, *scratch, *raw_f, *tmp_level, *tmp_level2;
};
static size_t carve_forward(const rnerf_model* m, int32_t B, bool own_path, void* ws, FwdBuffers* f) {
  Carver c(ws);
  const size_t Nc = m->num_coarse, Nf = m->num_fine, N = Nc * (size_t)m->num_path, S = Nc + Nf;
  f->path_pd = own_path ? c.take<float>(N * B * 4) : nullptr;
  f->path_dr = own_path ? c.take<float>(N * B * 4) : nullptr;
  f->bk_dirs = c.take<float>((size_t)B * 4);
  f->bkgd = c.take<float>((size_t)B * 3);
  f->raw_c = c.take<float>(Nc * B * 4);
  f->weights = c.take<float>(Nc * B);
  f->u = f->rows_pd = f->rows_dr = f->scratch = f->raw_f = f->tmp_level = f->tmp_level2 = nullptr;
  if (Nf > 0) {
    f->u = c.take<float>(Nf * (size_t)B);
    f->rows_pd = c.take<float>(S * B * 4);
    f->rows_dr = c.take<float>(S * B * 4);
    f->scratch = c.take<float>(S * B);
    f->raw_f = c.take<float>(S * B * 4);
    if (m->bd_cut) { f->tmp_level = c.take<float>((size_t)RNERF_LEVEL_FLOATS * B); f->tmp_level2 = c.take<float>((size_t)RNERF_LEVEL_FLOATS * B); }
  }
  return (c.off + 255) & ~(size_t)255;
}

static int check_model(const rnerf_model* m, int32_t B, const char* who) {
  RNERF_CHECK_ARG(m, "%s: null model", who);
  RNERF_CHECK_ARG(m->table, "%s: model.table is null", who);
  RNERF_CHECK_ARG(B >= 1, "%s: B must be >= 1", who);
  RNERF_CHECK_ARG(m->num_coarse >= 3 && m->num_fine >= 0 && m->num_path >= 1, "%s: need num_coarse >= 3, num_fine >= 0, num_path >= 1", who);
  RNERF_CHECK_ARG((long long)m->num_coarse * m->num_path >= 2, "%s: need at least two eikonal nodes", who);
  return RNERF_OK;
}

static inline int level_mask_mode(const rnerf_model* m) { return m->bd_cut == 2 ? 3 : 0; }
static inline const double* level_mask_box(const rnerf_model* m) { return m->bd_cut == 2 ? m->bd_cut_bbox : nullptr; }
struct Level { float *rgb, *dist, *acc, *trans, *tb; };
static Level level_of(float* out, int32_t B) { return Level{out, out + 3 * (size_t)B, out + 4 * (size_t)B, out + 5 * (size_t)B, out + 6 * (size_t)B}; }

static int bd_cut_pair(const rnerf_model* m, const float* raw_f, const float* rows_pd, const float* rows_dr, int32_t S, int32_t B, const float* bkgd,
                       Level out, float* tmp1, float* tmp2, void* stream) {
  Level a = level_of(tmp1, B), b = level_of(tmp2, B);
  int rc = rnerf_composite(raw_f, rows_pd, rows_dr, nullptr, S, B, nullptr, m->white_bkgd, m->rgb_padding, m->sigma_bias, a.rgb, a.dist, a.acc, out.trans,
                           a.tb, nullptr, nullptr, 1, m->bd_cut_bbox, stream);
  if (rc) return rc;
  rc = rnerf_composite(raw_f, rows_pd, rows_dr, nullptr, S, B, bkgd, m->white_bkgd, m->rgb_padding, m->sigma_bias, b.rgb, b.dist, b.acc, b.trans, b.tb, nullptr,
                       nullptr, 2, m->bd_cut_bbox, stream);
  if (rc) return rc;
  hipLaunchKernelGGL(bd_cut_mul_kernel, dim3((3 * B + 255) / 256), dim3(256), 0, (hipStream_t)stream, out.trans, b.rgb, B, out.tb);
  RNERF_CHECK_LAUNCH();
  return RNERF_OK;
}

static int make_u(const rnerf_model* m, int32_t B, int randomized, const uint32_t* key_u_dev, float* u, int32_t* per_ray, void* stream) {
  const double eps = 1.1920928955078125e-07;
  if (randomized) {
    *per_ray = 1;
    return rnerf_stratified_u_dev(key_u_dev, B, m->num_fine, u, stream);
  }
  *per_ray = 0;
  hipLaunchKernelGGL(linspace_u_kernel, dim3((m->num_fine + 255) / 256), dim3(256), 0, (hipStream_t)stream, m->num_fine, 1.0 - eps, u);
  RNERF_CHECK_LAUNCH();
  return RNERF_OK;
}

}

using namespace rnerf;

#define RNERF_TRY(expr)        \
  do {                         \
    int rc_ = (expr);          \
    if (rc_ != RNERF_OK) return rc_; \
  } while (0)

extern "C" int rnerf_rng_split3(uint32_t* rng_state, uint32_t* keys4, void* stream) {
  RNERF_CHECK_ARG(rng_state && keys4, "rnerf_rng_split3: null pointer");
  hipLaunchKernelGGL(rng_split3_kernel, dim3(1), dim3(64), 0, (hipStream_t)stream, rng_state, keys4);
  RNERF_CHECK_LAUNCH();
  return RNERF_OK;
}

extern "C" int rnerf_rng_forward(const uint32_t* keys4, int32_t num_coarse, int32_t num_path, int32_t use_random_choice, int32_t* jitter, uint32_t* key_u,
                                 void* stream) {
  RNERF_CHECK_ARG(keys4 && jitter, "rnerf_rng_forward: null pointer");
  RNERF_CHECK_ARG(num_coarse >= 1 && num_path >= 1, "rnerf_rng_forward: need num_coarse >= 1 and num_path >= 1");
  hipLaunchKernelGGL(rng_forward_kernel, dim3((num_coarse + 255) / 256), dim3(256), 0, (hipStream_t)stream, keys4, num_coarse, num_path, use_random_choice,
                     jitter, key_u);
  RNERF_CHECK_LAUNCH();
  return RNERF_OK;
}

extern "C" int rnerf_stratified_u_dev(const uint32_t* key_dev, int32_t B, int32_t num_fine, float* u, void* stream) {
  RNERF_CHECK_ARG(key_dev && u, "rnerf_stratified_u_dev: null pointer");
  RNERF_CHECK_ARG(B >= 1 && num_fine >= 1, "rnerf_stratified_u_dev: need B >= 1 and num_fine >= 1");
  const double eps = 1.1920928955078125e-07, s = 1.0 / num_fine;
  const long long half = ((long long)B * num_fine + 1) / 2;
  hipLaunchKernelGGL(stratified_u_dev_kernel, dim3((unsigned)((half + 255) / 256)), dim3(256), 0, (hipStream_t)stream, key_dev, B, num_fine, (float)s,
                     (float)(s - eps), (float)(1.0 - eps), u);
  RNERF_CHECK_LAUNCH();
  return RNERF_OK;
}

extern "C" size_t rnerf_forward_workspace_bytes(const rnerf_model* m, int32_t B) {
  if (!m || B < 1) return 0;
  FwdBuffers f;
  return carve_forward(m, B, true, nullptr, &f);
}

extern "C" int rnerf_forward(const rnerf_model* m, const float* origins, const float* viewdirs, int32_t B, const int32_t* jitter, const float* u_fine,
                             int32_t u_per_ray, const float* path_pd, const float* path_dr, float* out_coarse, float* out_fine, void* workspace,
                             int32_t max_workgroups, void* stream) {
  RNERF_TRY(check_model(m, B, "rnerf_forward"));
  RNERF_CHECK_ARG(jitter && out_coarse && workspace, "rnerf_forward: null pointer");
  RNERF_CHECK_ARG((path_pd == nullptr) == (path_dr == nullptr), "rnerf_forward: give both path_pd and path_dr or neither");
  RNERF_CHECK_ARG(path_pd || (origins && viewdirs), "rnerf_forward: origins / viewdirs are null and no marched path was given");
  RNERF_CHECK_ARG(m->packed_coarse && m->bkgd_params, "rnerf_forward: model.packed_coarse / bkgd_params are null");
  RNERF_CHECK_ARG(m->num_fine == 0 || (m->packed_fine && out_fine && u_fine), "rnerf_forward: num_fine > 0 needs packed_fine, out_fine and u_fine");
  RNERF_CHECK_ARG(((uintptr_t)workspace & 255) == 0, "rnerf_forward: workspace must be 256-byte aligned");
  const int32_t Nc = m->num_coarse, Nf = m->num_fine, N = Nc * m->num_path, S = Nc + Nf;
  FwdBuffers f;
  carve_forward(m, B, path_pd == nullptr, workspace, &f);
  if (!path_pd) {
    RNERF_TRY(rnerf_march(m->table, &m->grid, origins, viewdirs, B, m->near, m->far, N, f.path_pd, f.path_dr, nullptr, nullptr, stream));
    path_pd = f.path_pd; path_dr = f.path_dr;
  }
  hipStream_t st = (hipStream_t)stream;
  hipLaunchKernelGGL(bkgd_dirs_kernel, dim3((B + 255) / 256), dim3(256), 0, st, (const float4*)path_dr, jitter, Nc, B, (const float*)nullptr, 0, (float4*)f.bk_dirs);
  RNERF_CHECK_LAUNCH();
  RNERF_TRY(rnerf_bkgd_forward(m->bkgd_params, f.bk_dirs, 4, B, m->rgb_padding, f.bkgd, stream));
  RNERF_TRY(rnerf_nerfmlp_forward(m->packed_coarse, m->precision, path_pd, path_dr, jitter, Nc, B, f.raw_c, max_workgroups, stream));
  Level c = level_of(out_coarse, B);
  RNERF_TRY(rnerf_composite(f.raw_c, path_pd, path_dr, jitter, Nc, B, f.bkgd, m->white_bkgd, m->rgb_padding, m->sigma_bias, c.rgb, c.dist, c.acc, c.trans, c.tb,
                            Nf > 0 ? f.weights : nullptr, nullptr, level_mask_mode(m), level_mask_box(m), stream));
  if (Nf > 0) {
    RNERF_TRY(rnerf_resample(path_pd, path_dr, N, B, jitter, Nc, f.weights, u_fine, u_per_ray, Nf, f.rows_pd, f.rows_dr, nullptr, f.scratch, stream));
    RNERF_TRY(rnerf_nerfmlp_forward(m->packed_fine, m->precision, f.rows_pd, f.rows_dr, nullptr, S, B, f.raw_f, max_workgroups, stream));
    Level o = level_of(out_fine, B);
    RNERF_TRY(rnerf_composite(f.raw_f, f.rows_pd, f.rows_dr, nullptr, S, B, f.bkgd, m->white_bkgd, m->rgb_padding, m->sigma_bias, o.rgb, o.dist, o.acc, o.trans,
                              o.tb, nullptr, nullptr, level_mask_mode(m), level_mask_box(m), stream));
    if (m->bd_cut == 1) RNERF_TRY(bd_cut_pair(m, f.raw_f, f.rows_pd, f.rows_dr, S, B, f.bkgd, o, f.tmp_level, f.tmp_level2, stream));
  }
  return RNERF_OK;
}

namespace rnerf {
static bool levels_side_by_side(const rnerf_model* m, const rnerf_train_cfg* c, int32_t B) {
  if (m->num_fine <= 0 || !c->aux_stream) return false;
  const int cus = current_device_cus();
  const long long tiles_both = ((long long)m->num_coarse * B + 255) / 256 + ((long long)(m->num_coarse + m->num_fine) * B + 255) / 256;
  return tiles_both <= 2LL * cus;
}
struct TrainBuffers {
  FwdBuffers f;
  int32_t* jitter; uint32_t* key_u;
  void *packed_c, *packed_f, *packed_bwd, *packed_bwd_f, *save_c, *save_f, *save_bk, *dy, *dy_bk, *wgrad_ws;
  void *dy_c, *wgrad_ws_c;
  float *out_all, *level_c, *level_f, *sums, *d_all, *d_raw, *env_sum, *d_raw_c;
};
static size_t carve_train(const rnerf_model* m, const rnerf_train_cfg* c, int32_t B, bool own_path, void* ws, TrainBuffers* t) {
  const size_t Nc = m->num_coarse, Nf = m->num_fine, S = Nc + Nf;
  const size_t M = c->bg_smooth_weight > 0 ? (size_t)c->bg_patch_size * c->bg_patch_size : 0;
  Carver k(ws);
  const size_t N = Nc * (size_t)m->num_path;
  FwdBuffers& f = t->f;
  f.path_pd = own_path ? k.take<float>(N * B * 4) : nullptr;
  f.path_dr = own_path ? k.take<float>(N * B * 4) : nullptr;
  f.bk_dirs = k.take<float>((B + M) * 4);
  t->out_all = k.take<float>((B + M) * 3);
  f.bkgd = t->out_all;
  f.raw_c = k.take<float>(Nc * B * 4);
  f.weights = k.take<float>(Nc * B);
  f.u = f.rows_pd = f.rows_dr = f.scratch = f.raw_f = f.tmp_level = f.tmp_level2 = nullptr;
  if (Nf > 0) {
    f.u = k.take<float>(Nf * (size_t)B);
    f.rows_pd = k.take<float>(S * B * 4);
    f.rows_dr = k.take<float>(S * B * 4);
    f.scratch = k.take<float>(S * B);
    f.raw_f = k.take<float>(S * B * 4);
    if (m->bd_cut) { f.tmp_level = k.take<float>((size_t)RNERF_LEVEL_FLOATS * B); f.tmp_level2 = k.take<float>((size_t)RNERF_LEVEL_FLOATS * B); }
  }
  t->jitter = k.take<int32_t>(Nc);
  t->key_u = k.take<uint32_t>(4);
  t->packed_c = k.bytes(rnerf_nerfmlp_packed_bytes(RNERF_PREC_F16X3));
  t->packed_f = Nf > 0 ? k.bytes(rnerf_nerfmlp_packed_bytes(RNERF_PREC_F16X3)) : nullptr;
  t->packed_bwd = k.bytes(rnerf_nerfmlp_bwd_packed_bytes());
  t->packed_bwd_f = Nf > 0 ? k.bytes(rnerf_nerfmlp_bwd_packed_bytes()) : nullptr;
  t->save_c = k.bytes(rnerf_nerfmlp_save_bytes((int64_t)Nc * B, c->backward));
  t->save_f = Nf > 0 ? k.bytes(rnerf_nerfmlp_save_bytes((int64_t)S * B, c->backward)) : nullptr;
  t->save_bk = k.bytes(rnerf_bkgd_save_bytes((int64_t)(B + M)));
  t->dy = k.bytes(rnerf_nerfmlp_dy_bytes((int64_t)S * B, c->backward));
  t->dy_bk = k.bytes(rnerf_bkgd_dy_bytes((int64_t)(B + M)));
  t->wgrad_ws = k.bytes(rnerf_nerfmlp_wgrad_workspace_bytes());
  t->level_c = k.take<float>((size_t)RNERF_LEVEL_FLOATS * B);
  t->level_f = Nf > 0 ? k.take<float>((size_t)RNERF_LEVEL_FLOATS * B) : nullptr;
  t->sums = k.take<float>(4);
  t->env_sum = k.take<float>(rnerf_env_smooth_sum_floats(c->bg_smooth_weight > 0 ? c->bg_patch_size : 0));
  t->d_all = k.take<float>((B + M) * 3);
  t->d_raw = k.take<float>(S * B * 4);
  t->dy_c = t->wgrad_ws_c = nullptr; t->d_raw_c = nullptr;
  if (levels_side_by_side(m, c, B)) {
    t->dy_c = k.bytes(rnerf_nerfmlp_dy_bytes((int64_t)Nc * B, c->backward));
    t->wgrad_ws_c = k.bytes(rnerf_nerfmlp_wgrad_workspace_bytes());
    t->d_raw_c = k.take<float>(Nc * B * 4);
  }
  return (k.off + 255) & ~(size_t)255;
}
}

extern "C" size_t rnerf_train_workspace_bytes(const rnerf_model* m, const rnerf_train_cfg* c, int32_t B) {
  if (!m || !c || B < 1) return 0;
  TrainBuffers t;
  return carve_train(m, c, B, true, nullptr, &t);
}

static int mark_point(hipStream_t first, hipEvent_t* out);
static int wait_point(hipStream_t then, hipEvent_t e);

extern "C" int rnerf_train_forward_backward(const rnerf_model* m, const rnerf_train_cfg* c, const float* theta, const float* origins, const float* viewdirs,
                                            const float* pixels, const float* env_dirs, int32_t B, const uint32_t* keys4, const int32_t* jitter_override,
                                            const float* u_override, int32_t u_per_ray, const float* path_pd, const float* path_dr, float* grads,
                                            void* workspace, int32_t max_workgroups, const rnerf_prefetch* next, void* stream) {
  RNERF_TRY(check_model(m, B, "rnerf_train_forward_backward"));
  RNERF_CHECK_ARG(c && theta && pixels && grads && workspace, "rnerf_train_forward_backward: null pointer");
  RNERF_CHECK_ARG(keys4 || (jitter_override && (m->num_fine == 0 || u_override || !c->randomized)),
                  "rnerf_train_forward_backward: give keys4, or the jitter (and the stratified draws) explicitly");
  RNERF_CHECK_ARG((path_pd == nullptr) == (path_dr == nullptr), "rnerf_train_forward_backward: give both path_pd and path_dr or neither");
  RNERF_CHECK_ARG(path_pd || (origins && viewdirs), "rnerf_train_forward_backward: origins / viewdirs are null and no marched path was given");
  RNERF_CHECK_ARG(m->precision == RNERF_PREC_F16X3 || (m->precision == RNERF_PREC_F16 && c->backward != RNERF_BWD_F16X3 && c->backward != RNERF_BWD_F16X3_LO8) ||
                      (m->precision == RNERF_PREC_BF16X3 && c->backward == RNERF_BWD_BF16),
                  "rnerf_train_forward_backward: training is built on the f16x3 forward (f16: with backward f16 / bf16 only; bf16x3 + backward bf16: the range-safe step)");
  RNERF_CHECK_ARG(((uintptr_t)workspace & 255) == 0, "rnerf_train_forward_backward: workspace must be 256-byte aligned");
  const bool smooth = c->bg_smooth_weight > 0;
  RNERF_CHECK_ARG(!smooth || (env_dirs && c->bg_patch_size >= 2), "rnerf_train_forward_backward: bg_smooth_weight > 0 needs env_dirs and bg_patch_size >= 2");
  const int32_t Nc = m->num_coarse, Nf = m->num_fine, N = Nc * m->num_path, S = Nc + Nf;
  const int32_t ps = smooth ? c->bg_patch_size : 0, M = ps * ps;
  const int bwd = c->backward, prec = m->precision;
  hipStream_t st = (hipStream_t)stream;
  TrainBuffers t;
  carve_train(m, c, B, path_pd == nullptr, workspace, &t);
  FwdBuffers& f = t.f;
  const float* th_c = theta;
  const float* th_f = Nf > 0 ? theta + RNERF_NERFMLP_PARAMS : nullptr;
  const float* th_b = theta + (size_t)RNERF_NERFMLP_PARAMS * (Nf > 0 ? 2 : 1);
  const int64_t n_theta = (int64_t)RNERF_NERFMLP_PARAMS * (Nf > 0 ? 2 : 1) + RNERF_BKGDMLP_PARAMS;
  float* g_c = grads;
  float* g_f = Nf > 0 ? grads + RNERF_NERFMLP_PARAMS : nullptr;
  float* g_b = grads + (size_t)RNERF_NERFMLP_PARAMS * (Nf > 0 ? 2 : 1);
  float* stats8 = grads + n_theta;

  void* aux = c->aux_stream;
  bool pre_zeroed = false;
  struct Mark { hipEvent_t e = nullptr; ~Mark() { if (e) pool_put(e); } } fine_packed;
  if (aux) {
    RNERF_TRY(rnerf_fork(stream, aux));
    void* streams[2] = {t.packed_c, t.packed_f};
    void* dys[2] = {t.dy, t.dy_c};
    const int64_t dy_rows[2] = {(int64_t)(Nf > 0 ? S : Nc) * B, (int64_t)Nc * B};
    RNERF_TRY(nerfmlp_step_zero(prec, streams, Nf > 0 ? 2 : 1, bwd, dys, dy_rows, t.dy_c ? 2 : 1, (hipStream_t)aux));
    pre_zeroed = true;
    RNERF_TRY(nerfmlp_pack_impl(th_c, prec, t.packed_c, false, (hipStream_t)aux, false));
  }
  const int32_t* jitter = jitter_override;
  if (keys4) {
    RNERF_TRY(rnerf_rng_forward(keys4, Nc, m->num_path, c->use_random_choice, t.jitter, t.key_u, stream));
    if (!jitter_override) jitter = t.jitter;
  }
  if (!path_pd) {
    RNERF_TRY(rnerf_march(m->table, &m->grid, origins, viewdirs, B, m->near, m->far, N, f.path_pd, f.path_dr, nullptr, nullptr, stream));
    path_pd = f.path_pd; path_dr = f.path_dr;
  }
  hipLaunchKernelGGL(bkgd_dirs_kernel, dim3((B + M + 255) / 256), dim3(256), 0, st, (const float4*)path_dr, jitter, Nc, B, env_dirs, M, (float4*)f.bk_dirs);
  RNERF_CHECK_LAUNCH();
  RNERF_TRY(rnerf_bkgd_forward_train(th_b, f.bk_dirs, 4, (int64_t)B + M, m->rgb_padding, t.out_all, t.save_bk, stream));
  const float* bkgd = t.out_all;
  const float* rgb_env = t.out_all + (size_t)3 * B;
  if (aux) {
    RNERF_TRY(rnerf_join(stream, aux));
    if (Nf > 0) {
      RNERF_TRY(nerfmlp_pack_impl(th_f, prec, t.packed_f, false, (hipStream_t)aux, false));
      RNERF_TRY(mark_point((hipStream_t)aux, &fine_packed.e));
    }
    RNERF_CHECK_HIP(hipMemsetAsync(grads, 0, (size_t)(n_theta + 8) * sizeof(float), (hipStream_t)aux));
    RNERF_TRY(rnerf_nerfmlp_pack_bwd(th_c, bwd, t.packed_bwd, aux));
    if (Nf > 0) RNERF_TRY(rnerf_nerfmlp_pack_bwd(th_f, bwd, t.packed_bwd_f, aux));
    RNERF_TRY(rnerf_theta_sumsq(theta, n_theta, stats8, aux));
  } else {
    RNERF_TRY(rnerf_nerfmlp_pack(th_c, prec, t.packed_c, stream));
  }
  RNERF_TRY(rnerf_nerfmlp_forward_train(t.packed_c, prec, path_pd, path_dr, jitter, Nc, B, f.raw_c, t.save_c, bwd, max_workgroups, stream));
  Level lc = level_of(t.level_c, B);
  RNERF_TRY(rnerf_composite(f.raw_c, path_pd, path_dr, jitter, Nc, B, bkgd, m->white_bkgd, m->rgb_padding, m->sigma_bias, lc.rgb, lc.dist, lc.acc, lc.trans, lc.tb,
                            Nf > 0 ? f.weights : nullptr, nullptr, level_mask_mode(m), level_mask_box(m), stream));
  Level lf = lc;
  if (Nf > 0) {
    const float* u = u_override;
    int32_t per_ray = u_per_ray;
    if (!u) { RNERF_TRY(make_u(m, B, c->randomized, t.key_u, f.u, &per_ray, stream)); u = f.u; }
    RNERF_TRY(rnerf_resample(path_pd, path_dr, N, B, jitter, Nc, f.weights, u, per_ray, Nf, f.rows_pd, f.rows_dr, nullptr, f.scratch, stream));
    if (!aux) RNERF_TRY(rnerf_nerfmlp_pack(th_f, prec, t.packed_f, stream));
    else { hipEvent_t e = fine_packed.e; fine_packed.e = nullptr; RNERF_TRY(wait_point(st, e)); }
    RNERF_TRY(rnerf_nerfmlp_forward_train(t.packed_f, prec, f.rows_pd, f.rows_dr, nullptr, S, B, f.raw_f, t.save_f, bwd, max_workgroups, stream));
    lf = level_of(t.level_f, B);
    RNERF_TRY(rnerf_composite(f.raw_f, f.rows_pd, f.rows_dr, nullptr, S, B, bkgd, m->white_bkgd, m->rgb_padding, m->sigma_bias, lf.rgb, lf.dist, lf.acc, lf.trans,
                              lf.tb, nullptr, nullptr, level_mask_mode(m), level_mask_box(m), stream));
    if (m->bd_cut == 1) RNERF_TRY(bd_cut_pair(m, f.raw_f, f.rows_pd, f.rows_dr, S, B, bkgd, lf, f.tmp_level, f.tmp_level2, stream));
  }
  RNERF_TRY(rnerf_loss_reduce(Nf > 0 ? lc.rgb : nullptr, lf.rgb, lf.trans, lf.tb, pixels, B, t.sums, stream));
  const double bg_on = (c->bg_weight > 0 && c->annealed_alpha > 0) ? 1.0 : 0.0;
  const double mse_scale = 2.0 / (3.0 * B);
  const double env_on = c->annealed_alpha > 0 ? 1.0 : 0.0;
  if (!aux) RNERF_CHECK_HIP(hipMemsetAsync(grads, 0, (size_t)(n_theta + 8) * sizeof(float), st));
  auto march_next = [&]() -> int {
    RNERF_CHECK_ARG(next->origins && next->viewdirs && next->path_pd && next->path_dr && next->side_stream, "rnerf_train_forward_backward: incomplete rnerf_prefetch");
    RNERF_TRY(rnerf_fork(stream, next->side_stream));
    return rnerf_march(m->table, &m->grid, next->origins, next->viewdirs, B, m->near, m->far, N, next->path_pd, next->path_dr, nullptr, nullptr,
                       next->side_stream);
  };
  if (aux) RNERF_TRY(rnerf_join(stream, aux));
  float* d_first = t.d_all;
  const bool split_levels = levels_side_by_side(m, c, B);
  float* d_raw_c = split_levels ? t.d_raw_c : t.d_raw;
  void* dy_c = split_levels ? t.dy_c : t.dy;
  if (Nf > 0) {
    RNERF_TRY(rnerf_composite_backward(f.raw_f, f.rows_pd, f.rows_dr, nullptr, S, B, bkgd, m->rgb_padding, m->sigma_bias, lf.rgb, pixels, lf.trans, lf.tb, t.sums,
                                       mse_scale, c->bg_weight * bg_on, t.d_raw, d_first, 0, m->white_bkgd, m->bd_cut == 1 ? 1 : level_mask_mode(m), m->bd_cut ? m->bd_cut_bbox : nullptr, stream));
    if (split_levels) {
      RNERF_TRY(rnerf_composite_backward(f.raw_c, path_pd, path_dr, jitter, Nc, B, bkgd, m->rgb_padding, m->sigma_bias, lc.rgb, pixels, nullptr, nullptr, nullptr,
                                         mse_scale, 0.0, d_raw_c, d_first, 1, m->white_bkgd, level_mask_mode(m), level_mask_box(m), stream));
      RNERF_TRY(rnerf_fork(stream, aux));
      if (smooth) RNERF_TRY(rnerf_env_smooth_backward(rgb_env, ps, c->bg_smooth_weight * env_on, t.d_all + (size_t)3 * B, t.env_sum, aux));
      RNERF_TRY(rnerf_bkgd_backward(th_b, t.save_bk, t.d_all, (int64_t)B + M, m->rgb_padding, t.dy_bk, g_b, nullptr, aux));
      RNERF_TRY(nerfmlp_dgrad_impl(t.packed_bwd, t.packed_c, prec, bwd, t.save_c, d_raw_c, (int64_t)Nc * B, dy_c, !pre_zeroed, false, (hipStream_t)aux));
      RNERF_TRY(rnerf_nerfmlp_wgrad(prec, bwd, t.save_c, dy_c, (int64_t)Nc * B, g_c, t.wgrad_ws_c, aux));
    }
    if (!aux) RNERF_TRY(rnerf_nerfmlp_pack_bwd(th_f, bwd, t.packed_bwd_f, stream));
    RNERF_TRY(nerfmlp_dgrad_impl(t.packed_bwd_f, t.packed_f, prec, bwd, t.save_f, t.d_raw, (int64_t)S * B, t.dy, !pre_zeroed, !split_levels, st));
    if (next) RNERF_TRY(march_next());
    RNERF_TRY(rnerf_nerfmlp_wgrad(prec, bwd, t.save_f, t.dy, (int64_t)S * B, g_f, t.wgrad_ws, stream));
    if (split_levels)
      RNERF_TRY(rnerf_join(stream, aux));
    else
      RNERF_TRY(rnerf_composite_backward(f.raw_c, path_pd, path_dr, jitter, Nc, B, bkgd, m->rgb_padding, m->sigma_bias, lc.rgb, pixels, nullptr, nullptr, nullptr,
                                         mse_scale, 0.0, t.d_raw, d_first, 1, m->white_bkgd, level_mask_mode(m), level_mask_box(m), stream));
  } else {
    RNERF_TRY(rnerf_composite_backward(f.raw_c, path_pd, path_dr, jitter, Nc, B, bkgd, m->rgb_padding, m->sigma_bias, lf.rgb, pixels, lf.trans, lf.tb, t.sums,
                                       mse_scale, c->bg_weight * bg_on, t.d_raw, d_first, 0, m->white_bkgd, level_mask_mode(m), level_mask_box(m), stream));
  }
  if (!aux) RNERF_TRY(rnerf_nerfmlp_pack_bwd(th_c, bwd, t.packed_bwd, stream));
  if (!split_levels)
    RNERF_TRY(nerfmlp_dgrad_impl(t.packed_bwd, t.packed_c, prec, bwd, t.save_c, t.d_raw, (int64_t)Nc * B, t.dy, !(pre_zeroed && Nf == 0), true, st));
  if (next && Nf == 0) RNERF_TRY(march_next());
  const bool tail_on_aux = aux && !split_levels;
  void* tail = tail_on_aux ? aux : stream;
  if (tail_on_aux) RNERF_TRY(rnerf_fork(stream, aux));
  if (!split_levels && !tail_on_aux) RNERF_TRY(rnerf_nerfmlp_wgrad(prec, bwd, t.save_c, t.dy, (int64_t)Nc * B, g_c, t.wgrad_ws, stream));
  if (!tail_on_aux && c->grads_stream) RNERF_TRY(rnerf_fork(stream, c->grads_stream));
  if (!split_levels) {
    if (smooth) RNERF_TRY(rnerf_env_smooth_backward(rgb_env, ps, c->bg_smooth_weight * env_on, t.d_all + (size_t)3 * B, t.env_sum, tail));
    RNERF_TRY(rnerf_bkgd_backward(th_b, t.save_bk, t.d_all, (int64_t)B + M, m->rgb_padding, t.dy_bk, g_b, nullptr, tail));
  }
  RNERF_TRY(rnerf_train_stats(t.sums, B, Nf > 0, c->bg_weight * bg_on, smooth ? t.env_sum : nullptr, ps, env_on, aux ? nullptr : theta, n_theta, c->frozen_sq,
                              n_theta + c->frozen_count, stats8, tail));
  if (tail_on_aux) {
    RNERF_TRY(rnerf_nerfmlp_wgrad(prec, bwd, t.save_c, t.dy, (int64_t)Nc * B, g_c, t.wgrad_ws, stream));
    if (c->grads_stream) RNERF_TRY(rnerf_fork(stream, c->grads_stream));
    RNERF_TRY(rnerf_join(stream, aux));
  }
  return RNERF_OK;
}

static int adam_update_impl(const rnerf_adam_cfg* c, float* theta, float* mu, float* nu, float* grads, int64_t n_theta, const float* frozen_params,
                            int64_t n_frozen, int32_t* step_counter, float* scratch, bool fused, float* count_out, hipStream_t st) {
  const double wd2 = c->weight_decay_mult > 0 ? 2.0 * c->weight_decay_mult / (double)c->n_all : 0.0;
  const int want_norm = c->grad_max_norm > 0;
  float* scal = scratch;
  float* partial = scratch + 4;
  float* bad_partial = nullptr;
  int n_partial = 0;
  if (wd2 != 0.0 || c->grad_max_val > 0 || want_norm || c->skip_nonfinite) {
    bad_partial = scratch + 4 + 2 * ADAM_BLOCKS;
    hipLaunchKernelGGL(adam_prep_kernel, dim3(ADAM_BLOCKS), dim3(256), 0, st, (const float*)theta, grads, (long long)n_theta, (float)wd2, (float)c->grad_max_val,
                       want_norm, partial, bad_partial, fused ? step_counter : nullptr);
    if (want_norm) {
      n_partial = ADAM_BLOCKS;
      if (frozen_params && n_frozen > 0 && wd2 != 0.0) {
        hipLaunchKernelGGL(adam_frozen_sq_kernel, dim3(ADAM_BLOCKS), dim3(256), 0, st, frozen_params, (long long)n_frozen, (float)wd2, (float)c->grad_max_val,
                           partial + ADAM_BLOCKS);
        n_partial = 2 * ADAM_BLOCKS;
      }
    }
  }
  AdamSched s{c->lr_init, c->lr_final, c->lr_delay_mult, (double)c->max_steps, (double)c->lr_delay_steps, c->b1, c->b2, c->grad_max_norm, c->lr_override, c->use_lr_override != 0,
              c->skip_nonfinite != 0};
  if (fused && bad_partial) {
    hipLaunchKernelGGL(adam_apply_fused_kernel, dim3(ADAM_BLOCKS), dim3(256), 0, st, s, (const int*)step_counter, (const float*)partial, n_partial,
                       (const float*)bad_partial, theta, mu, nu, (const float*)grads, (long long)n_theta, (float)c->b1, (float)c->b2, (float)c->eps, scal, count_out);
    RNERF_CHECK_LAUNCH();
    return RNERF_OK;
  }
  hipLaunchKernelGGL(adam_scalars_kernel, dim3(1), dim3(256), 0, st, s, step_counter, (const float*)partial, n_partial, (const float*)bad_partial, scal);
  hipLaunchKernelGGL(adam_apply_kernel, dim3(ADAM_BLOCKS), dim3(256), 0, st, theta, mu, nu, (const float*)grads, (long long)n_theta, (float)c->b1, (float)c->b2,
                     (float)c->eps, scal, bad_partial == nullptr);
  RNERF_CHECK_LAUNCH();
  if (count_out) RNERF_CHECK_HIP(hipMemcpyAsync(count_out, scal + 3, sizeof(float), hipMemcpyDefault, st));
  return RNERF_OK;
}

extern "C" int rnerf_adam_update(const rnerf_adam_cfg* c, float* theta, float* mu, float* nu, float* grads, int64_t n_theta, const float* frozen_params,
                                 int64_t n_frozen, int32_t* step_counter, float* scratch, void* stream) {
  RNERF_CHECK_ARG(c && theta && mu && nu && grads && step_counter && scratch, "rnerf_adam_update: null pointer");
  RNERF_CHECK_ARG(n_theta >= 1 && c->n_all >= n_theta, "rnerf_adam_update: need n_theta >= 1 and n_all >= n_theta");
  return adam_update_impl(c, theta, mu, nu, grads, n_theta, frozen_params, n_frozen, step_counter, scratch, false, nullptr, (hipStream_t)stream);
}

extern "C" int rnerf_adam_update_fused(const rnerf_adam_cfg* c, float* theta, float* mu, float* nu, float* grads, int64_t n_theta, const float* frozen_params,
                                       int64_t n_frozen, int32_t* step_counter, float* scratch, float* nonfinite_out, void* stream) {
  RNERF_CHECK_ARG(c && theta && mu && nu && grads && step_counter && scratch, "rnerf_adam_update_fused: null pointer");
  RNERF_CHECK_ARG(n_theta >= 1 && c->n_all >= n_theta, "rnerf_adam_update_fused: need n_theta >= 1 and n_all >= n_theta");
  return adam_update_impl(c, theta, mu, nu, grads, n_theta, frozen_params, n_frozen, step_counter, scratch, true, nonfinite_out, (hipStream_t)stream);
}

namespace {
std::mutex g_ev_mu;
thread_local std::vector<hipEvent_t> tl_capture_events;
std::vector<std::pair<void*, std::vector<hipEvent_t>>> g_graph_events;
void drop_events(std::vector<hipEvent_t>& v) {
  for (hipEvent_t e : v) (void)hipEventDestroy(e);
  v.clear();
}
}

extern "C" int rnerf_graph_begin(void* stream) {
  drop_events(tl_capture_events);
  RNERF_CHECK_HIP(hipStreamBeginCapture((hipStream_t)stream, hipStreamCaptureModeThreadLocal));
  return RNERF_OK;
}

extern "C" int rnerf_graph_end(void* stream, void** graph_exec) {
  RNERF_CHECK_ARG(graph_exec, "rnerf_graph_end: null pointer");
  hipGraph_t g = nullptr;
  hipError_t err = hipStreamEndCapture((hipStream_t)stream, &g);
  if (err != hipSuccess) { drop_events(tl_capture_events); set_error("hipStreamEndCapture failed: %s", hipGetErrorString(err)); return RNERF_ERR_HIP; }
  hipGraphExec_t e = nullptr;
  err = hipGraphInstantiate(&e, g, nullptr, nullptr, 0);
  hipGraphDestroy(g);
  if (err != hipSuccess) { drop_events(tl_capture_events); set_error("hipGraphInstantiate failed: %s", hipGetErrorString(err)); return RNERF_ERR_HIP; }
  {
    std::lock_guard<std::mutex> l(g_ev_mu);
    g_graph_events.emplace_back((void*)e, std::move(tl_capture_events));
  }
  tl_capture_events.clear();
  *graph_exec = (void*)e;
  return RNERF_OK;
}

extern "C" int rnerf_graph_launch(void* graph_exec, void* stream) {
  RNERF_CHECK_ARG(graph_exec, "rnerf_graph_launch: null graph");
  RNERF_CHECK_HIP(hipGraphLaunch((hipGraphExec_t)graph_exec, (hipStream_t)stream));
  return RNERF_OK;
}

extern "C" int rnerf_graph_destroy(void* graph_exec) {
  if (!graph_exec) return RNERF_OK;
  std::vector<hipEvent_t> ev;
  {
    std::lock_guard<std::mutex> l(g_ev_mu);
    for (size_t i = 0; i < g_graph_events.size(); ++i)
      if (g_graph_events[i].first == graph_exec) { ev = std::move(g_graph_events[i].second); g_graph_events.erase(g_graph_events.begin() + i); break; }
  }
  RNERF_CHECK_HIP(hipGraphExecDestroy((hipGraphExec_t)graph_exec));
  drop_events(ev);
  return RNERF_OK;
}

static int order_after(hipStream_t first, hipStream_t then) {
  hipEvent_t e = nullptr;
  RNERF_CHECK_HIP(pool_get(&e));
  hipStreamCaptureStatus cs = hipStreamCaptureStatusNone;
  hipError_t err = hipStreamIsCapturing(first, &cs);
  if (err == hipSuccess) err = hipEventRecord(e, first);
  if (err == hipSuccess) err = hipStreamWaitEvent(then, e, 0);
  if (err != hipSuccess) {
    (void)hipEventDestroy(e);
    set_error("stream ordering failed: %s", hipGetErrorString(err));
    return RNERF_ERR_HIP;
  }
  if (cs == hipStreamCaptureStatusNone) pool_put(e);
  else tl_capture_events.push_back(e);
  return RNERF_OK;
}

static int mark_point(hipStream_t first, hipEvent_t* out) {
  hipEvent_t e = nullptr;
  RNERF_CHECK_HIP(pool_get(&e));
  const hipError_t err = hipEventRecord(e, first);
  if (err != hipSuccess) { (void)hipEventDestroy(e); set_error("stream ordering failed: %s", hipGetErrorString(err)); return RNERF_ERR_HIP; }
  *out = e;
  return RNERF_OK;
}
static int wait_point(hipStream_t then, hipEvent_t e) {
  hipStreamCaptureStatus cs = hipStreamCaptureStatusNone;
  hipError_t err = hipStreamIsCapturing(then, &cs);
  if (err == hipSuccess) err = hipStreamWaitEvent(then, e, 0);
  if (err != hipSuccess) { (void)hipEventDestroy(e); set_error("stream ordering failed: %s", hipGetErrorString(err)); return RNERF_ERR_HIP; }
  if (cs == hipStreamCaptureStatusNone) pool_put(e);
  else tl_capture_events.push_back(e);
  return RNERF_OK;
}

extern "C" int rnerf_fork(void* main_stream, void* side_stream) { return order_after((hipStream_t)main_stream, (hipStream_t)side_stream); }
extern "C" int rnerf_join(void* main_stream, void* side_stream) { return order_after((hipStream_t)side_stream, (hipStream_t)main_stream); }
```

### samplenerfro_amd/train.py

```python
from __future__ import annotations

import contextlib
import ctypes as C
import os
import weakref
from typing import Any, Dict, Optional

import numpy as np
import torch

from . import _lib, distributed, ops, prng
from .models import BKGD_MLP_SHAPES, NERF_MLP_SHAPES, SO3_MLP_SHAPES, NerfModel, make_variables
from .utils import Rays, Stats, learning_rate_decay

_RANGE_RETRY_LAG = 2
_LAG_SLOTS = 8
_SKIP_NONFINITE_UPDATES = True

_N_STATS = 8


class TrainState:

    def __init__(self, step, theta, mu, nu, variables, segments, lr_fn, flags=None):
# ... 34 lines not shown
        stage = getattr(flags, "stage", "radiance")
        if stage.startswith("all"):
            names.append("so3_mlp")
        elif stage.startswith("ior"):
            names = ["so3_mlp"]
        shapes = {"coarse_mlp": NERF_MLP_SHAPES, "fine_mlp": NERF_MLP_SHAPES, "bkgd_mlp": BKGD_MLP_SHAPES, "so3_mlp": SO3_MLP_SHAPES}
        parts = [model._flat(variables, n, shapes[n]).detach().reshape(-1).float() for n in names]
        theta = torch.cat(parts).contiguous()
        segments, off = {}, 0
        flat = dict(variables.get("flat", {}))
        for n, p in zip(names, parts):
            segments[n] = (off, off + p.numel())
            flat[n] = theta[off:off + p.numel()]
            off += p.numel()
        new_vars = make_variables(flat)
        lr_fn = lambda count: learning_rate_decay(count, flags.lr_init, flags.lr_final, flags.max_steps, flags.lr_delay_steps,
                                                  flags.lr_delay_mult)
        return cls(0, theta, torch.zeros_like(theta), torch.zeros_like(theta), new_vars, segments, lr_fn, flags)

    def grad_view(self, name: str) -> torch.Tensor:
        lo, hi = self.segments[name]
        return self.grads[lo:hi]

    def apply_gradients(self, grads: torch.Tensor, b1: float = 0.9, b2: float = 0.999, eps: float = 1e-8) -> "TrainState":
        count = self.step
        lr = self.lr_fn(count)
        t = count + 1
        self.mu.mul_(b1).add_(grads, alpha=1 - b1)
        self.nu.mul_(b2).addcmul_(grads, grads, value=1 - b2)
        denom = (self.nu / (1 - b2 ** t)).sqrt_().add_(eps)
        self.theta.addcdiv_(self.mu, denom, value=-lr / (1 - b1 ** t))
        self.step = t
        return self

    def state_dict(self) -> Dict[str, Any]:
        if self._lag_pending:
            model = self._model_ref() if self._model_ref is not None else None
            if model is None:
                raise RuntimeError("TrainState.state_dict(): steps of range_retry='lag' are still pending and their model is gone; "
                                   "call flush_range_retry(model, state) before reading the parameters")
            flush_range_retry(model, self)
        return {"step": self.step, "theta": self.theta, "mu": self.mu, "nu": self.nu}

    def restore_flax(self, state: Dict[str, Any]) -> "TrainState":
        from .checkpoint import find_params, flat_from_params
        flat = flat_from_params(find_params(state), self.theta.device, tuple(self.segments))
        for name, (lo, hi) in self.segments.items():
            self.theta[lo:hi].copy_(flat[name])
        self.step = int(state.get("step", 0))
        try:
            adam = state["opt_state"]["inner_states"]["adam_lr_scheduler"]["inner_state"]["0"]
            for which, buf in (("mu", self.mu), ("nu", self.nu)):
                m = flat_from_params(adam[which]["params"], self.theta.device, tuple(self.segments))
                for name, (lo, hi) in self.segments.items():
                    buf[lo:hi].copy_(m[name])
        except (KeyError, TypeError, ValueError):
            pass
        frozen = flat_from_params(find_params(state), self.theta.device, ("so3_mlp",)) if "so3_mlp" not in self.segments else {}
        cur = self.variables.get("flat", {}).get("so3_mlp")
        if "so3_mlp" in frozen and cur is not None:
            cur.copy_(frozen["so3_mlp"])
        self.frozen_sq = None
        return self

    def load_state_dict(self, d: Dict[str, Any]) -> None:
        self._lag_pending.clear()
        self.step = int(d["step"])
        for k in ("theta", "mu", "nu"):
            getattr(self, k).copy_(d[k])
        self.frozen_sq = None


def _bwd_packed(model: NerfModel, state: TrainState, name: str, backward: int) -> torch.Tensor:
    cache = model.__dict__.setdefault("_packed_bwd", {})
    flat = state.variables["flat"][name]
    ent = cache.get(name)
    if ent is None or ent[0]() is not flat or ent[1] != flat._version or ent[3] != backward:
        buf = ops.nerfmlp_pack_bwd(flat, ent[2] if ent is not None else None, backward)
        cache[name] = (weakref.ref(flat), flat._version, buf, backward)
    return cache[name][2]


def backward_mode(flags, model: NerfModel) -> int:
    name = getattr(flags, "backward_precision", "f16x3")
    if name not in _lib.BACKWARDS:
        raise ValueError(f"backward_precision must be one of {sorted(_lib.BACKWARDS)}")
    mode = _lib.BACKWARDS[name]
    if model.precision == _lib.PREC_BF16X3 and mode == _lib.BWD_BF16:
        return mode
    if model.precision != _lib.PREC_F16X3 and not (model.precision == _lib.PREC_F16 and mode not in _lib.TWO_PLANE_BACKWARDS):
        raise ValueError('training is built on the f16x3 forward (NerfModel(precision="f16x3")), or — one MFMA per product, the north-star '
                         'arithmetic as a labelled leg — on the f16 forward with backward_precision "f16" / "bf16"; the other precisions are inference modes')
    return mode


def _ior_stage_step(model: NerfModel, rng, state: TrainState, batch, flags):
    rng, _key_0, _key_1 = prng.split(np.asarray(rng, np.uint32), 3)
    annealed = float(np.asarray(batch["annealed_alpha"]).reshape(-1)[0])
    variables = state.variables
    others = [v for k, v in variables["flat"].items() if k not in state.segments]
    n_all = state.theta.numel() + sum(int(v.numel()) for v in others)
    sq = (state.theta.double() ** 2).sum() + sum((v.double() ** 2).sum() for v in others)
    weight_l2 = (sq / n_all).float()
    grads = state.grads[:state.theta.numel()]
    grads.copy_(state.theta).mul_(2.0 * flags.weight_decay_mult / n_all)
    distributed.allreduce_mean_([grads])
    if flags.grad_max_val > 0:
        grads.clamp_(-flags.grad_max_val, flags.grad_max_val)
    if flags.grad_max_norm > 0:
        og = [v * (2.0 * flags.weight_decay_mult / n_all) for v in others]
        if flags.grad_max_val > 0:
            og = [v.clamp(-flags.grad_max_val, flags.grad_max_val) for v in og]
        norm = torch.sqrt((grads * grads).sum() + sum((v * v).sum() for v in og))
        grads.mul_(torch.clamp(flags.grad_max_norm / (1e-7 + norm), max=1.0))
    state.apply_gradients(grads)
    zero = torch.zeros((), device=state.theta.device)
    stats = Stats(loss=zero, psnr=zero, loss_c=zero, psnr_c=zero, weight_l2=weight_l2, loss_sp=0.0, loss_nrm=0.0, annealing_rate=annealed,
                  coarse_alpha_target=0.0, fine_alpha_target=0.0, loss_bg=zero, loss_bg_c=0.0, loss_bg_smooth=0.0)
    return state, stats, rng


def _all_stage_backward(model: NerfModel, state: TrainState, variables, ctx, dy_c, d_bk_dirs, bwd: int, annealed: float, taps) -> None:
    B, Nc, N = ctx["B"], model.num_coarse_samples, model.num_samples
    rec = ops.finalize_pairs(ctx["march_rec"])
    coarse_flat = variables["flat"]["coarse_mlp"]
    so3_flat = variables["flat"]["so3_mlp"]
    a_pos, a_dir = ops.nerfmlp_input_grad(coarse_flat, bwd, dy_c, ctx["path_pd"], ctx["path_dr"], ctx["jit"], Nc, B)
    a_dir[Nc - 1] += d_bk_dirs[:B]
    sample_of_node = torch.full((N,), -1, dtype=torch.int32, device=a_pos.device)
    sample_of_node[ctx["jit"].long()] = torch.arange(Nc, dtype=torch.int32, device=a_pos.device)
    n = rec["n_pairs"]
    if n > 0:
        raw, save = ops.so3_forward_train(so3_flat, rec["window"], rec["pair_x"])
        eye = torch.zeros((3 * n, 4), dtype=torch.float32, device=a_pos.device)
        for j in range(3):
            eye[j * n:(j + 1) * n, j] = 1.0
        J = ops.so3_backward(so3_flat, rec["window"], rec["pair_x"], save, eye)
        A, P = ops.so3_pair_jacobian(model.table, model.spec, rec["pair_x"], rec["pair_g"], raw.contiguous(), J)
    else:
        A = P = torch.zeros((1, 12), dtype=torch.float32, device=a_pos.device)
    v = ops.march_adjoint(model.table, model.spec, rec, A, P, a_pos, a_dir, sample_of_node, model.near, model.far)
    if n > 0:
        ops.so3_backward(so3_flat, rec["window"], rec["pair_x"], save, v, grads=state.grad_view("so3_mlp"), want_dx=False)
    if taps is not None:
        taps.update(a_pos=a_pos, a_dir=a_dir, n_pairs=n, v_pairs=v)


def frozen_sq_of(state: TrainState, variables):
    so3 = variables.get("flat", {}).get("so3_mlp") if "so3_mlp" not in state.segments else None
    fkey = (id(so3), so3._version) if so3 is not None else None
    if state.frozen_sq is None or state.frozen_sq[2] != fkey or (so3 is not None and state.frozen_sq[3]() is not so3):
        state.frozen_sq = (float((so3.double() ** 2).sum()) if so3 is not None else 0.0, so3.numel() if so3 is not None else 0, fkey,
                           weakref.ref(so3) if so3 is not None else None)
    return state.frozen_sq


def train_cfg(model: NerfModel, state: TrainState, flags, annealed: float) -> "_lib.TrainCfg":
    c = _lib.TrainCfg()
    c.backward = backward_mode(flags, model)
    c.randomized, c.use_random_choice = int(bool(flags.randomized)), int(model.use_random_choice)
    c.bg_patch_size = int(flags.bg_patch_size) if flags.bg_smooth_weight > 0 else 0
    c.bg_weight, c.bg_smooth_weight, c.annealed_alpha = float(flags.bg_weight), float(flags.bg_smooth_weight), float(annealed)
    fs = frozen_sq_of(state, state.variables)
    c.frozen_sq, c.frozen_count = fs[0], fs[1]
    c.aux_stream = model.tail_stream().cuda_stream
    return c


def adam_cfg(state: TrainState, flags, lr_override: Optional[float] = None) -> "_lib.AdamCfg":
    a = _lib.AdamCfg()
    a.lr_init, a.lr_final, a.lr_delay_mult = float(flags.lr_init), float(flags.lr_final), float(flags.lr_delay_mult)
    a.max_steps, a.lr_delay_steps = int(flags.max_steps), int(flags.lr_delay_steps)
    a.b1, a.b2, a.eps = 0.9, 0.999, 1e-8
    a.weight_decay_mult, a.grad_max_val, a.grad_max_norm = float(flags.weight_decay_mult), float(flags.grad_max_val), float(flags.grad_max_norm)
    a.n_all = state.theta.numel() + frozen_sq_of(state, state.variables)[1]
    a.use_lr_override = int(lr_override is not None)
    a.lr_override = float(lr_override) if lr_override is not None else 0.0
    a.skip_nonfinite = int(_SKIP_NONFINITE_UPDATES)
    return a


def _adam_update_on_device(state: TrainState, flags) -> None:
    lib = _lib.load()
    default_lr = state._lr_fn_default is state.lr_fn
    a = adam_cfg(state, flags, None if default_lr else float(state.lr_fn(state.step)))
    state.sync_step_counter()
    fs = frozen_sq_of(state, state.variables)
    frozen = state.variables["flat"].get("so3_mlp") if fs[1] > 0 else None
    word = getattr(state, "_lag_word", None)
    _lib.check(lib.rnerf_adam_update_fused(C.byref(a), state.theta.data_ptr(), state.mu.data_ptr(), state.nu.data_ptr(), state.grads.data_ptr(),
                                           state.theta.numel(), _lib.ptr(frozen), fs[1], state.step_dev.data_ptr(), state.adam_scratch.data_ptr(),
                                           word, _lib.current_stream()), "rnerf_adam_update_fused")
    if word is not None:
        state._lag_word_written = True
    state.step += 1
    state._step_dev_value = state.step
    state._staged_bad = None
    _bump(state.theta)


def _train_step_whole(model: NerfModel, rng, state: TrainState, batch, flags, jitter, u_fine, path, next_rays):
    lib = _lib.load()
    rng, key_0, key_1 = prng.split(np.asarray(rng, np.uint32), 3)
    annealed = float(np.asarray(batch["annealed_alpha"]).reshape(-1)[0])
    rays: Rays = batch["rays"]
    o, v = ops._chk(rays.origins, "origins"), ops._chk(rays.viewdirs, "viewdirs")
    pixels = ops._chk(batch["pixels"][..., :3].contiguous(), "pixels")
    B = o.shape[0]
    env = None
    if flags.bg_smooth_weight > 0:
        env = ops._chk(batch["env_rays"].viewdirs.reshape(-1, 3), "env_rays.viewdirs")
        if env.shape[0] != flags.bg_patch_size ** 2:
            raise ValueError("env_rays.viewdirs must hold bg_patch_size^2 directions")
    m = model.c_model()
    c = train_cfg(model, state, flags, annealed)
    st = _lib.current_stream()
    keys = model._keys_dev(key_0, key_1)
    jit = model._jitter_dev(jitter) if jitter is not None else None
    u, per_ray = None, 0
    if u_fine is not None:
        u = ops._chk(u_fine, "u_fine"); per_ray = 1 if u.dim() == 2 else 0
    pd = dr = None
    if path is not None:
        if path.batch != B:
            raise ValueError("path handle was marched for a different batch size")
        cur = torch.cuda.current_stream()
        cur.wait_event(path.event)
        pd, dr = path.pd, path.dr
        pd.record_stream(cur); dr.record_stream(cur)
    ws = model._workspace("train", lib.rnerf_train_workspace_bytes(C.byref(m), C.byref(c), B))
    G = state.grads
    n_theta = state.theta.numel()
    nxt, next_path = None, None
    if next_rays is not None:
        next_path, nxt = model.prefetch_slot(next_rays)
    comm = model.comm_stream() if (distributed.active() and hasattr(model, "comm_stream")) else None
    if comm is not None:
        c = _lib.TrainCfg.from_buffer_copy(c)
        c.grads_stream = comm.cuda_stream
    _lib.check(lib.rnerf_train_forward_backward(C.byref(m), C.byref(c), state.theta.data_ptr(), o.data_ptr(), v.data_ptr(), pixels.data_ptr(), _lib.ptr(env), B,
                                                keys.data_ptr(), _lib.ptr(jit), _lib.ptr(u), per_ray, _lib.ptr(pd), _lib.ptr(dr), G.data_ptr(), ws.data_ptr(),
                                                int(model._mlp_wg_limit), C.byref(nxt) if nxt is not None else None, st), "rnerf_train_forward_backward")
    if next_path is not None:
        next_path.event.record(model._side)
    if comm is not None:
        n_big = state.segments["bkgd_mlp"][0]
        with torch.cuda.stream(comm):
            pending = distributed.allreduce_begin(G[:n_big])
        distributed.allreduce_mean_([G[n_big:]])
        distributed.allreduce_end_mean_(pending, G[:n_big])
    else:
        distributed.allreduce_mean_([G])
    _adam_update_on_device(state, flags)
    s8 = G[n_theta:]
    two = model.num_fine_samples > 0
    stats = Stats(loss=s8[0], psnr=s8[6], loss_c=s8[1], psnr_c=(s8[7] if two else 0.0), weight_l2=s8[4], loss_sp=0.0, loss_nrm=0.0,
                  annealing_rate=annealed, coarse_alpha_target=0.0, fine_alpha_target=0.0, loss_bg=s8[2], loss_bg_c=0.0,
                  loss_bg_smooth=s8[3])
    state.next_path = next_path
    return state, stats, rng


def _bump(t: torch.Tensor) -> None:
    try:
        torch._C._autograd._unsafe_set_version_counter([t], [t._version + 1])
    except (AttributeError, TypeError):
        t.add_(0)


@contextlib.contextmanager
def range_safe(model: NerfModel, flags):
    saved = (model.precision, model._packed, getattr(flags, "backward_precision", "f16x3"))
    model.precision, model._packed, flags.backward_precision = _lib.PREC_BF16X3, {}, "bf16"
    try:
        yield model
    finally:
        model.precision, model._packed, flags.backward_precision = saved


_F16_BASED = (_lib.PREC_F16X3, _lib.PREC_F16)


def train_step(model: NerfModel, rng, state: TrainState, batch: Dict[str, Any], flags=None, *, range_retry=None, **kw):
    flags = state.flags if flags is None else flags
    mode = getattr(flags, "range_retry", False) if range_retry is None else range_retry
    retry = bool(mode)
    if not (retry and flags.stage.startswith("radiance") and model.precision in _F16_BASED):
        return _train_step_once(model, rng, state, batch, flags, **kw)
    if mode == "lag":
        if kw.get("taps") is not None or kw.get("forward_taps") is not None or torch.cuda.is_current_stream_capturing():
            return _train_step_once(model, rng, state, batch, flags, **kw)
        ctx = _dist_context()
        slot = state._lag_count % _LAG_SLOTS
        state._lag_count += 1
        state._lag_word, state._lag_word_written = state._lag_host[slot:slot + 1].data_ptr(), False
        try:
            out = _train_step_once(model, rng, state, batch, flags, **kw)
        finally:
            state._lag_word = None
        if not state._lag_word_written:
            state._lag_host[slot:slot + 1].copy_(state.adam_scratch[3:4], non_blocking=True)
        ev = torch.cuda.Event(); ev.record()
        replay = dict(kw, next_rays=None, path=None)
        state._lag_pending.append((ev, slot, rng, _clone_batch(batch), flags, replay, ctx))
        state._model_ref = weakref.ref(model)
        while len(state._lag_pending) > _RANGE_RETRY_LAG:
            pend = state._lag_pending.pop(0)
            if _lag_flag(state, pend):
                out = (out[0], _clone_stats(out[1]), out[2])
            _settle_lagged(model, state, pend)
        return out
    step0 = state.step
    out = _train_step_once(model, rng, state, batch, flags, _guard=True, **kw)
    if state.nonfinite_grads() == 0:
        return out
    next_path = state.next_path
    state.step = step0
    state.sync_step_counter()
    kw = dict(kw, next_rays=None)
    with range_safe(model, flags):
        out = _train_step_once(model, rng, state, batch, flags, _guard=True, **kw)
    state.next_path = next_path
    _count_rerun(state)
    return out


def _dist_context():
    return (distributed._GROUP, bool(distributed._skip()))


@contextlib.contextmanager
def _in_dist_context(ctx):
    saved = (distributed._GROUP, distributed._SKIP)
    distributed._GROUP, distributed._SKIP = ctx
    try:
        yield
    finally:
        distributed._GROUP, distributed._SKIP = saved


def _clone_batch(batch: Dict[str, Any]) -> Dict[str, Any]:
    srcs = []

    def walk(v):
        if isinstance(v, torch.Tensor):
            if v.is_cuda and v.dtype == torch.float32:
                srcs.append(v)
                return ("t", len(srcs) - 1)
            return ("c", v.clone())
        if isinstance(v, tuple) and hasattr(v, "_fields"):
            return ("n", type(v), [walk(x) for x in v])
        return ("c", v)

    plan = {k: walk(v) for k, v in batch.items()}
    views = []
    if srcs:
        offs, total = [], 0
        for t in srcs:
            offs.append(total)
            total += (t.numel() + 63) // 64 * 64
        flat = torch.empty(total, dtype=torch.float32, device=srcs[0].device)
        views = [flat[o:o + t.numel()].view(t.shape) for o, t in zip(offs, srcs)]
        torch._foreach_copy_(views, [t if t.is_contiguous() else t.contiguous() for t in srcs])

    def build(node):
        if node[0] == "t":
            return views[node[1]]
        if node[0] == "n":
            return node[1](*[build(x) for x in node[2]])
        return node[1]
    return {k: build(v) for k, v in plan.items()}


def _clone_stats(stats: Stats) -> Stats:
    import dataclasses
    return dataclasses.replace(stats, **{f.name: getattr(stats, f.name).clone() for f in dataclasses.fields(stats)
                                         if isinstance(getattr(stats, f.name), torch.Tensor)})


def _count_rerun(state: TrainState) -> None:
    state.range_retries += 1
    if state.nonfinite_grads() != 0:
        state.range_retry_failures += 1
        import warnings
        warnings.warn("train_step: the range-safe re-run of a skipped batch has a non-finite gradient too; its update stays skipped "
                      f"({state.range_retry_failures} so far)", RuntimeWarning, stacklevel=3)


def _lag_flag(state: TrainState, pending) -> bool:
    pending[0].synchronize()
    return float(state._lag_host[pending[1]]) != 0.0


def _settle_lagged(model: NerfModel, state: TrainState, pending) -> None:
    ev, slot, rng, batch, flags, replay, ctx = pending
    if not _lag_flag(state, pending):
        return
    next_path = state.next_path
    state.step -= 1
    state.sync_step_counter()
    with range_safe(model, flags), _in_dist_context(ctx):
        _, stats, _ = _train_step_once(model, rng, state, batch, flags, **replay)
    state.next_path = next_path
    state.last_retry_stats = _clone_stats(stats)
    _count_rerun(state)


def flush_range_retry(model: NerfModel, state: TrainState) -> None:
    while state._lag_pending:
        _settle_lagged(model, state, state._lag_pending.pop(0))


def _train_step_once(model: NerfModel, rng, state: TrainState, batch: Dict[str, Any], flags=None, *, jitter=None, u_fine=None,
                     taps: Optional[dict] = None, path=None, next_rays: Optional[Rays] = None, forward_taps: Optional[dict] = None,
                     noise_c=None, noise_f=None, _guard: bool = False):
    flags = state.flags if flags is None else flags
    all_stage = flags.stage.startswith("all")
    if flags.stage.startswith("ior"):
        return _ior_stage_step(model, rng, state, batch, flags)
    if not (flags.stage.startswith("radiance") or all_stage):
        raise NotImplementedError(f"train_step: unknown stage {flags.stage!r}")
    if all_stage and model.stage != flags.stage:
        raise ValueError("stage all*: build the model with the same stage (the march must evaluate so3_mlp)")
    if flags.beta_weight > 0 or flags.sparsity_weight > 0:
        pass
    noisy = getattr(model, "noise_std", None) is not None and bool(flags.randomized)
    if not all_stage and taps is None and forward_taps is None and getattr(model, "whole_path", False) and not noisy:
        return _train_step_whole(model, rng, state, batch, flags, jitter, u_fine, path, next_rays)
    rng, key_0, key_1 = prng.split(np.asarray(rng, np.uint32), 3)
    annealed = float(np.asarray(batch["annealed_alpha"]).reshape(-1)[0])
    rays: Rays = batch["rays"]
    pixels = batch["pixels"][..., :3].contiguous()
    variables = state.variables
    prec = model.precision
    if all_stage and next_rays is not None:
        if model._side is None:
            from .models import shared_stream
            model._side = shared_stream(model.device, "march")
        ops.prefetch_shell_order(model.table, model.spec, next_rays.origins, next_rays.viewdirs, model.near, model.far, model.num_samples, model._side)
        next_rays = None
    Nc, Nf = model.num_coarse_samples, model.num_fine_samples
    bwd = backward_mode(flags, model)
    if all_stage and bwd == _lib.BWD_BF16:
        raise ValueError('stage all*: the input gradients are built on the row-normalised backward modes (backward_precision "f16x3" or "f16")')
    ctx: Dict[str, Any] = {"backward": bwd, "loss_sp": taps is not None}
    if flags.bg_smooth_weight > 0:
        ev = batch["env_rays"].viewdirs
        ctx["env_dirs"] = ev.reshape(-1, 3)
    ret, _loss_sp = model.apply(variables, key_0, key_1, rays, flags.randomized, annealed, jitter=jitter, u_fine=u_fine, ctx=ctx, path=path,
                             taps=forward_taps, noise_c=noise_c, noise_f=noise_f)
    B = ctx["B"]
    rgb_f, _, _, trans_f, tb_f = ret[-1]
    rgb_c = ret[0][0] if len(ret) > 1 else None
    sums = ops.loss_reduce(rgb_c, rgb_f, trans_f, tb_f, pixels)
    bg_on = 1.0 if (flags.bg_weight > 0 and annealed > 0) else 0.0
    mse_scale = 2.0 / (3.0 * B)

    G = state.grads
    G.zero_()
    M_env = ctx["rgb_env"].shape[0] if flags.bg_smooth_weight > 0 else 0
    d_all = torch.empty((B + M_env, 3), dtype=torch.float32, device=pixels.device)
    d_first = d_all[:B]
    if Nf > 0:
        d_raw_f, d_bkgd = ops.composite_backward(ctx["raw_f"], ctx["rows_pd"], ctx["rows_dr"], None, Nc + Nf, B, ctx["bkgd"], rgb_f, pixels,
                                                 trans_f, tb_f, sums, mse_scale, flags.bg_weight * bg_on, rgb_padding=model.rgb_padding,
                                                 sigma_bias=model.sigma_bias, bd_cut_bbox=ctx.get("bd_cut_bbox"), white_bkgd=model.white_bkgd,
                                                 d_bkgd=d_first, accumulate_bkgd=False, mask_bbox=ctx.get("mask_bbox"))
        ops.nerfmlp_backward(_bwd_packed(model, state, "fine_mlp", bwd), model._packed_weights(variables, "fine_mlp"), prec, ctx["save_f"],
                             d_raw_f, (Nc + Nf) * B, grads=state.grad_view("fine_mlp"), backward=bwd)
        d_raw_c, d_bkgd = ops.composite_backward(ctx["raw_c"], ctx["path_pd"], ctx["path_dr"], ctx["jit"], Nc, B, ctx["bkgd"], rgb_c, pixels,
                                                 None, None, None, mse_scale, 0.0, d_bkgd=d_bkgd, rgb_padding=model.rgb_padding,
                                                 sigma_bias=model.sigma_bias, white_bkgd=model.white_bkgd, mask_bbox=ctx.get("mask_bbox"))
    else:
        d_raw_c, d_bkgd = ops.composite_backward(ctx["raw_c"], ctx["path_pd"], ctx["path_dr"], ctx["jit"], Nc, B, ctx["bkgd"], rgb_f, pixels,
                                                 trans_f, tb_f, sums, mse_scale, flags.bg_weight * bg_on, rgb_padding=model.rgb_padding,
                                                 sigma_bias=model.sigma_bias, white_bkgd=model.white_bkgd, d_bkgd=d_first, accumulate_bkgd=False,
                                                 mask_bbox=ctx.get("mask_bbox"))
    if all_stage:
        dy_c = ops.nerfmlp_backward(_bwd_packed(model, state, "coarse_mlp", bwd), model._packed_weights(variables, "coarse_mlp"), prec, ctx["save_c"],
                                    d_raw_c, Nc * B, backward=bwd, stages="d")
    else:
        _, dy_c = ops.nerfmlp_backward(_bwd_packed(model, state, "coarse_mlp", bwd), model._packed_weights(variables, "coarse_mlp"), prec, ctx["save_c"],
                                       d_raw_c, Nc * B, grads=state.grad_view("coarse_mlp"), backward=bwd, return_dy=True)
    n_big = state.segments["bkgd_mlp"][0]
    pending = None if all_stage else distributed.allreduce_begin(G[:n_big])
    next_path = model.prefetch_path(next_rays, sync_inputs=True, reserve_cus=0) if next_rays is not None else None
    bk_flat = variables["flat"]["bkgd_mlp"]
    g_bk = state.grad_view("bkgd_mlp")
    ps, on, env_sum = 0, 0.0, None
    if flags.bg_smooth_weight > 0:
        ps = batch["env_rays"].viewdirs.shape[0]
        on = 1.0 if annealed > 0 else 0.0
        env_sum = torch.empty(_lib.load().rnerf_env_smooth_sum_floats(int(ps)), dtype=torch.float32, device=pixels.device)
        ops.env_smooth_backward(ctx["rgb_env"], ps, flags.bg_smooth_weight * on, d_all[B:], env_sum)
    if all_stage:
        _, d_bk_dirs = ops.bkgd_backward(bk_flat, ctx["save_bkgd"], d_all, g_bk, model.rgb_padding, want_d_dirs=True)
        main, side = torch.cuda.current_stream(), model.tail_stream()
        side.wait_stream(main)
        ops.nerfmlp_backward(_bwd_packed(model, state, "coarse_mlp", bwd), model._packed_weights(variables, "coarse_mlp"), prec, ctx["save_c"],
                             d_raw_c, Nc * B, grads=state.grad_view("coarse_mlp"), backward=bwd, dy=dy_c, stages="w")
        pending = distributed.allreduce_begin(G[:n_big])
        with torch.cuda.stream(side):
            _all_stage_backward(model, state, variables, ctx, dy_c, d_bk_dirs, bwd, annealed, taps)
        main.wait_stream(side)
    else:
        ops.bkgd_backward(bk_flat, ctx["save_bkgd"], d_all, g_bk, model.rgb_padding)
    n_theta = state.theta.numel()
    frozen_sq_of(state, variables)
    n_all = n_theta + state.frozen_sq[1]
    st = G[n_theta:]
    ops.train_stats(sums, B, rgb_c is not None, flags.bg_weight * bg_on, env_sum, ps, on, state.theta, state.frozen_sq[0], n_all, st)
    distributed.allreduce_mean_([G[n_big:]])
    distributed.allreduce_end_mean_(pending, G[:n_big])
    grads = G[:n_theta]
    if taps is None and state.adam_scratch is not None:
        _adam_update_on_device(state, flags)
        annealing_rate = 0.0
        stats = Stats(loss=st[0], psnr=st[6], loss_c=st[1], psnr_c=(st[7] if rgb_c is not None else 0.0),
                      weight_l2=st[4], loss_sp=flags.sparsity_weight * annealing_rate * _loss_sp, loss_nrm=0.0, annealing_rate=annealed, coarse_alpha_target=0.0,
                      fine_alpha_target=0.0, loss_bg=st[2], loss_bg_c=0.0, loss_bg_smooth=st[3])
        state.next_path = next_path
        return state, stats, rng
    if flags.weight_decay_mult > 0:
        grads.add_(state.theta, alpha=2.0 * flags.weight_decay_mult / n_all)
    if flags.grad_max_val > 0:
        grads.clamp_(-flags.grad_max_val, flags.grad_max_val)
    if flags.grad_max_norm > 0:
        sq = (grads * grads).sum()
        if flags.weight_decay_mult > 0 and state.frozen_sq[1] > 0:
            fg = variables["flat"]["so3_mlp"] * (2.0 * flags.weight_decay_mult / n_all)
            if flags.grad_max_val > 0:
                fg = fg.clamp(-flags.grad_max_val, flags.grad_max_val)
            sq = sq + (fg * fg).sum()
        norm = torch.sqrt(sq)
        grads.mul_(torch.clamp(flags.grad_max_norm / (1e-7 + norm), max=1.0))
    if taps is not None:
        taps.update(grads=grads.clone(), sums=sums, ctx=ctx, loss_sp=_loss_sp)
    state._staged_bad = None
    if _guard:
        state._staged_bad = int((~torch.isfinite(grads)).sum().item())
    if state._staged_bad:
        state.step += 1
    else:
        state.apply_gradients(grads)
    annealing_rate = 0.0
    stats = Stats(loss=st[0], psnr=st[6], loss_c=st[1], psnr_c=(st[7] if rgb_c is not None else 0.0),
                  weight_l2=st[4], loss_sp=flags.sparsity_weight * annealing_rate * _loss_sp, loss_nrm=0.0, annealing_rate=annealed, coarse_alpha_target=0.0, fine_alpha_target=0.0,
                  loss_bg=st[2], loss_bg_c=0.0, loss_bg_smooth=st[3])
    state.next_path = next_path
    return state, stats, rng
```

Measured before the change: 662,700.

## Split background MLP across four waves, vectorise wgrad reduce, and reorder side-stream work

The background MLP forward kernel now runs four waves per block, and each wave computes one 32-column output tile. Activations are exchanged through shared memory as split f16 planes, which cuts per-wave register pressure and weight loads but adds barriers and LDS traffic. The wgrad reduce kernel now handles four elements per thread with float4 loads and puts the bias reduction in a separate block range. The training pipeline reorders side-stream launches so the next march waits on an event after dgrad instead of forking, and the Python retry path clones batches on the aux stream.

```diff
diff --git a/samplenerfro_amd/csrc/bkgd16.hip b/samplenerfro_amd/csrc/bkgd16.hip
--- a/samplenerfro_amd/csrc/bkgd16.hip
+++ b/samplenerfro_amd/csrc/bkgd16.hip
@@ -83,12 +83,61 @@
     }
   });
 }
+template <int NS, bool FIRST, typename WF, typename LF, typename XF>
+__device__ __forceinline__ void bkgd16_tile_layer(f32x16& acc, WF wload, LF live, bool half0, XF xop) {
+  f32x2 w[NS][4];
+#pragma unroll
+  for (int s = 0; s < NS; ++s)
+#pragma unroll
+    for (int j = 0; j < 8; ++j)
+      if (live(s, j) != 0) w[s][j >> 1][j & 1] = wload(s, j);
+  f32x16 zero;
+#pragma unroll
+  for (int r = 0; r < 16; ++r) zero[r] = 0.f;
+  RNERF_PIN();
+#pragma unroll
+  for (int s = 0; s < NS; ++s) {
+    uint32_t hh[4], ll[4];
+#pragma unroll
+    for (int p = 0; p < 4; ++p) {
+      const int l0 = live(s, 2 * p), l1 = live(s, 2 * p + 1);
+      if (l0 == 0 && l1 == 0) { hh[p] = 0u; ll[p] = 0u; continue; }
+      f32x2 q = w[s][p];
+      if (l0 == 0) q[0] = 0.f;
+      if (l1 == 0) q[1] = 0.f;
+      q = q * 256.0f;
+      if (l0 == 2) q[0] = half0 ? q[0] : 0.f;
+      if (l1 == 2) q[1] = half0 ? q[1] : 0.f;
+      bkgd16_split2(q[0], q[1], hh[p], ll[p]);
+    }
+    const uint4 ah = make_uint4(hh[0], hh[1], hh[2], hh[3]), al = make_uint4(ll[0], ll[1], ll[2], ll[3]);
+    uint4 bh, bl;
+    xop(s, bh, bl);
+    acc = mfma16<true>(ah, bh, FIRST && s == 0 ? zero : acc);
+    acc = mfma16<true>(ah, bl, acc);
+    acc = mfma16<true>(al, bh, acc);
+  }
+}
+template <bool BIAS>
+__device__ __forceinline__ void bkgd16_prev_tile(f32x16& acc, const uint4* xs, int lane, const Bkgd16Lane& L, int koff, int boff) {
+  bkgd16_tile_layer<BIAS ? 9 : 8, true>(acc,
+      [&](int s, int j) { return s < 8 ? L.prev[koff + (16 * s + 8 * (j >> 2) + (j & 3)) * 128] : L.p0[boff]; },
+      [&](int s, int j) { return s < 8 ? 1 : (j == 0 ? 2 : 0); }, L.half0,
+      [&](int s, uint4& bh, uint4& bl) {
+    if (s < 8) {
+      bh = xs[(2 * s) * 64 + lane]; bl = xs[(2 * s + 1) * 64 + lane];
+    } else {
+      bh = make_uint4(L.half0 ? 0x3c00u : 0u, 0u, 0u, 0u);
+      bl = make_uint4(0u, 0u, 0u, 0u);
+    }
+  });
+}
 template <bool FIRST>
-__device__ __forceinline__ void bkgd16_dir_layer(f32x16 (&acc)[4], const float (&enc)[14], const Bkgd16Lane& L, int koff, int boff) {
-  bkgd16_layer<2, FIRST>(acc,
-      [&](int s, int t, int j) {
+__device__ __forceinline__ void bkgd16_dir_tile(f32x16& acc, const float (&enc)[14], const Bkgd16Lane& L, int koff, int boff) {
+  bkgd16_tile_layer<2, FIRST>(acc,
+      [&](int s, int j) {
         const int q = 8 * s + j;
-        return q < 12 ? L.dir[koff + (3 + q) * 128 + 32 * t] : (q == 12 ? L.sp[koff + 32 * t] : (q == 13 ? L.p0[koff + 128 + 32 * t] : L.p0[boff + 32 * t]));
+        return q < 12 ? L.dir[koff + (3 + q) * 128] : (q == 12 ? L.sp[koff] : (q == 13 ? L.p0[koff + 128] : L.p0[boff]));
       },
       [&](int s, int j) { const int q = 8 * s + j; return q < 13 ? 1 : (q < 15 ? 2 : 0); }, L.half0,
       [&](int s, uint4& bh, uint4& bl) {
@@ -100,10 +149,11 @@
 }
 
 template <bool TRAIN>
-__global__ void __launch_bounds__(64) bkgd16_fwd_kernel(const float* __restrict__ params, const float* __restrict__ dirs, int dir_stride,
-                                                        long long n, float pad_scale, float pad, float* __restrict__ out_rgb,
-                                                        float* __restrict__ save) {
-  const int lane = threadIdx.x & 63, m = lane & 31, h = lane >> 5;
+__global__ void __launch_bounds__(256) bkgd16_fwd_kernel(const float* __restrict__ params, const float* __restrict__ dirs, int dir_stride,
+                                                         long long n, float pad_scale, float pad, float* __restrict__ out_rgb,
+                                                         float* __restrict__ save) {
+  __shared__ uint4 xb[2][16 * 64];
+  const int lane = threadIdx.x & 63, m = lane & 31, h = lane >> 5, wv = threadIdx.x >> 6;
   long long row = (long long)blockIdx.x * 32 + m;
   const bool ok = row < n;
   if (!ok) row = n - 1;
@@ -118,54 +168,70 @@
   }
   enc[12] = h ? v2 : v0;
   enc[13] = h ? 0.f : v1;
-  auto save_x = [&](int k, const f32x16 (&xx)[4]) {
+  f32x16 acc, xt;
+  auto save_x = [&](int k) {
     if constexpr (TRAIN) {
       if (ok) {
         float* dst = save + (size_t)n * 28 + (size_t)(k - 1) * n * 128 + (size_t)row * 128;
 #pragma unroll
-        for (int t = 0; t < 4; ++t)
-#pragma unroll
-          for (int g = 0; g < 4; ++g)
-            *(float4*)(dst + 32 * t + 8 * g + 4 * h) = make_float4(xx[t][4 * g], xx[t][4 * g + 1], xx[t][4 * g + 2], xx[t][4 * g + 3]);
+        for (int g = 0; g < 4; ++g)
+          *(float4*)(dst + 32 * wv + 8 * g + 4 * h) = make_float4(xt[4 * g], xt[4 * g + 1], xt[4 * g + 2], xt[4 * g + 3]);
       }
     }
   };
   if constexpr (TRAIN) {
-    if (ok) {
+    if (ok && wv == 0) {
 #pragma unroll
       for (int q = 0; q < 14; ++q) { const int f = h ? dir_feature(q, 1) : dir_feature(q, 0); if (f >= 0) save[(size_t)row * 28 + f] = enc[q]; }
       if (h == 1) save[(size_t)row * 28 + 27] = 0.f;
     }
   }
   constexpr float INV = 1.0f / 256.0f;
-  f32x16 acc[4], x[4];
   auto relu_to_x = [&]() {
 #pragma unroll
-    for (int t = 0; t < 4; ++t)
-#pragma unroll
-      for (int r = 0; r < 16; ++r) { const float y = acc[t][r] * INV; x[t][r] = y < 0.f ? 0.f : y; }
-  };
-  const Bkgd16Lane L = bkgd16_lane(params, m, h);
-  bkgd16_dir_layer<true>(acc, enc, L, bkgd_koff(0), bkgd_boff(0));
-  relu_to_x();
-  save_x(1, x);
-  bkgd16_prev_layer<true>(acc, x, L, bkgd_koff(1), bkgd_boff(1));
-  relu_to_x();
-  save_x(2, x);
-  bkgd16_prev_layer<true>(acc, x, L, bkgd_koff(2), bkgd_boff(2));
-  relu_to_x();
-  save_x(3, x);
-  bkgd16_prev_layer<false>(acc, x, L, bkgd_koff(3), 0);
-  bkgd16_dir_layer<false>(acc, enc, L, bkgd_koff(3) + 128 * 128, bkgd_boff(3));
-  relu_to_x();
-  if constexpr (TRAIN) save_x(4, x);
+    for (int r = 0; r < 16; ++r) { const float y = acc[r] * INV; xt[r] = y < 0.f ? 0.f : y; }
+  };
+  auto publish = [&](int buf) {
+#pragma unroll
+    for (int a = 0; a < 2; ++a) {
+      float xv[8];
+#pragma unroll
+      for (int j = 0; j < 8; ++j) xv[j] = xt[8 * a + j];
+      uint4 bh, bl;
+      bkgd16_split8(xv, bh, bl);
+      xb[buf][(2 * (2 * wv + a)) * 64 + lane] = bh; xb[buf][(2 * (2 * wv + a) + 1) * 64 + lane] = bl;
+    }
+    __syncthreads();
+  };
+  const Bkgd16Lane L = bkgd16_lane(params, m + 32 * wv, h);
+  bkgd16_dir_tile<true>(acc, enc, L, bkgd_koff(0), bkgd_boff(0));
+  relu_to_x();
+  save_x(1);
+  publish(0);
+  bkgd16_prev_tile<true>(acc, xb[0], lane, L, bkgd_koff(1), bkgd_boff(1));
+  relu_to_x();
+  save_x(2);
+  publish(1);
+  bkgd16_prev_tile<true>(acc, xb[1], lane, L, bkgd_koff(2), bkgd_boff(2));
+  relu_to_x();
+  save_x(3);
+  publish(0);
+  bkgd16_prev_tile<false>(acc, xb[0], lane, L, bkgd_koff(3), 0);
+  bkgd16_dir_tile<false>(acc, enc, L, bkgd_koff(3) + 128 * 128, bkgd_boff(3));
+  relu_to_x();
+  if constexpr (TRAIN) save_x(4);
+  float* xf = (float*)xb[1];
+#pragma unroll
+  for (int r = 0; r < 16; ++r) xf[(16 * wv + r) * 64 + lane] = xt[r];
+  __syncthreads();
+  if (wv != 0) return;
   float o[3] = {0.f, 0.f, 0.f};
   const float* __restrict__ k4 = params + bkgd_koff(4);
 #pragma unroll
   for (int t = 0; t < 4; ++t)
 #pragma unroll
     for (int r = 0; r < 16; ++r) {
-      const float v = x[t][r];
+      const float v = xf[(16 * t + r) * 64 + lane];
       const int f = 32 * t + (r & 3) + 8 * (r >> 2) + 4 * h;
       o[0] = fmaf(v, k4[f * 3 + 0], o[0]); o[1] = fmaf(v, k4[f * 3 + 1], o[1]); o[2] = fmaf(v, k4[f * 3 + 2], o[2]);
     }
@@ -183,8 +249,8 @@
 static int launch_bkgd16_fwd(bool train, const float* params, const float* dirs, int dir_stride, long long n, float pad_scale, float pad, float* out_rgb,
                              float* save, hipStream_t st) {
   const dim3 grid((unsigned)((n + 31) / 32));
-  if (train) hipLaunchKernelGGL(bkgd16_fwd_kernel<true>, grid, dim3(64), 0, st, params, dirs, dir_stride, n, pad_scale, pad, out_rgb, save);
-  else hipLaunchKernelGGL(bkgd16_fwd_kernel<false>, grid, dim3(64), 0, st, params, dirs, dir_stride, n, pad_scale, pad, out_rgb, save);
+  if (train) hipLaunchKernelGGL(bkgd16_fwd_kernel<true>, grid, dim3(256), 0, st, params, dirs, dir_stride, n, pad_scale, pad, out_rgb, save);
+  else hipLaunchKernelGGL(bkgd16_fwd_kernel<false>, grid, dim3(256), 0, st, params, dirs, dir_stride, n, pad_scale, pad, out_rgb, save);
   RNERF_CHECK_LAUNCH();
   return RNERF_OK;
 }
diff --git a/samplenerfro_amd/csrc/mlp.hip b/samplenerfro_amd/csrc/mlp.hip
--- a/samplenerfro_amd/csrc/mlp.hip
+++ b/samplenerfro_amd/csrc/mlp.hip
@@ -1723,7 +1723,7 @@
 }
 
 __global__ void __launch_bounds__(256) wgrad_reduce_kernel(const float* __restrict__ workspace, const WgradTable tab, float* __restrict__ grads,
-                                                           const float* __restrict__ out_scale) {
+                                                           const float* __restrict__ out_scale, int elem_blocks) {
   const float osc = out_scale ? *out_scale : 1.0f;
   const int jb = blockIdx.y;
   const WgradJob job = tab.job[jb];
@@ -1731,7 +1731,6 @@
   const float* __restrict__ partial = workspace + tab.poff[jb];
   const float* __restrict__ partial_bias = workspace + tab.pboff[jb];
   const int ldn = job.NT * 32, rows = job.KT * 32;
-  const int e = blockIdx.x * blockDim.x + threadIdx.x;
   auto out_feature = [&](int J, int& dense) -> int {
     int nt = J >> 5;
     const int c = J & 31, a = c >> 4, hh = (c >> 3) & 1, j = c & 7;
@@ -1744,14 +1743,9 @@
     if (dkind == 1) return j == 0 ? 0 : -1;
     return (j >= 1 && j <= 3) ? j - 1 : -1;
   };
-  auto sum_over = [&](const float* __restrict__ p, size_t stride) -> float {
-    float s0 = 0.f, s1 = 0.f, s2 = 0.f, s3 = 0.f;
-    int g = 0;
-    for (; g + 4 <= n_wg; g += 4) { s0 += p[(size_t)g * stride]; s1 += p[(size_t)(g + 1) * stride]; s2 += p[(size_t)(g + 2) * stride]; s3 += p[(size_t)(g + 3) * stride]; }
-    for (; g < n_wg; ++g) s0 += p[(size_t)g * stride];
-    return (s0 + s1) + (s2 + s3);
-  };
-  if (e < rows * ldn) {
+  if ((int)blockIdx.x < elem_blocks) {
+    const int e = (blockIdx.x * blockDim.x + threadIdx.x) * 4;
+    if (e >= rows * ldn) return;
     const int I = e / ldn, J = e % ldn;
     int kt = I >> 5;
     const int c = I & 31, a = c >> 4, hh = (c >> 3) & 1, j = c & 7;
@@ -1760,13 +1754,49 @@
     if (segb) kt -= job.KTa;
     const int s = 2 * kt + a;
     int fin = xkind == 1 ? prev_feature(s, hh, j) : (xkind == 0 ? pe_feature(8 * s + j, hh) : view_feature(8 * s + j, hh));
-    int dense;
-    const int fout = out_feature(J, dense);
-    if (fin >= 0 && fout >= 0) {
-      fin += row_off;
-      if (fin < nerf_dense(dense).in) grads[nerf_koff(dense) + fin * nerf_dense(dense).out + fout] = sum_over(partial + e, (size_t)rows * ldn) * osc;
-    }
-  }
+    if (fin < 0) return;
+    fin += row_off;
+    int dense[4], fout[4];
+    bool any = false;
+#pragma unroll
+    for (int v = 0; v < 4; ++v) {
+      fout[v] = out_feature(J + v, dense[v]);
+      if (fout[v] >= 0 && fin >= nerf_dense(dense[v]).in) fout[v] = -1;
+      any = any || fout[v] >= 0;
+    }
+    if (!any) return;
+    const float4* __restrict__ p = (const float4*)(partial + e);
+    const size_t stride = (size_t)rows * ldn / 4;
+    float4 s0 = {0.f, 0.f, 0.f, 0.f}, s1 = s0, s2 = s0, s3 = s0;
+    auto add = [](float4& acc, const float4 v) { acc.x += v.x; acc.y += v.y; acc.z += v.z; acc.w += v.w; };
+    int g = 0;
+    for (; g + 8 <= n_wg; g += 8) {
+      float4 v[8];
+#pragma unroll
+      for (int u = 0; u < 8; ++u) v[u] = p[(size_t)(g + u) * stride];
+      add(s0, v[0]); add(s1, v[1]); add(s2, v[2]); add(s3, v[3]); add(s0, v[4]); add(s1, v[5]); add(s2, v[6]); add(s3, v[7]);
+    }
+    for (; g + 4 <= n_wg; g += 4) {
+      float4 v[4];
+#pragma unroll
+      for (int u = 0; u < 4; ++u) v[u] = p[(size_t)(g + u) * stride];
+      add(s0, v[0]); add(s1, v[1]); add(s2, v[2]); add(s3, v[3]);
+    }
+    for (; g < n_wg; ++g) add(s0, p[(size_t)g * stride]);
+    const float sum[4] = {(s0.x + s1.x) + (s2.x + s3.x), (s0.y + s1.y) + (s2.y + s3.y), (s0.z + s1.z) + (s2.z + s3.z), (s0.w + s1.w) + (s2.w + s3.w)};
+#pragma unroll
+    for (int v = 0; v < 4; ++v)
+      if (fout[v] >= 0) grads[nerf_koff(dense[v]) + fin * nerf_dense(dense[v]).out + fout[v]] = sum[v] * osc;
+    return;
+  }
+  auto sum_over = [&](const float* __restrict__ p, size_t stride) -> float {
+    float s0 = 0.f, s1 = 0.f, s2 = 0.f, s3 = 0.f;
+    int g = 0;
+    for (; g + 4 <= n_wg; g += 4) { s0 += p[(size_t)g * stride]; s1 += p[(size_t)(g + 1) * stride]; s2 += p[(size_t)(g + 2) * stride]; s3 += p[(size_t)(g + 3) * stride]; }
+    for (; g < n_wg; ++g) s0 += p[(size_t)g * stride];
+    return (s0 + s1) + (s2 + s3);
+  };
+  const int e = ((int)blockIdx.x - elem_blocks) * blockDim.x + threadIdx.x;
   if (job.write_bias && e < ldn) {
     int dense;
     const int fout = out_feature(e, dense);
@@ -2221,7 +2251,7 @@
     {SAVE_RGBIN, 8, DY_HEADS, 1, job1(11, 1, 0, 2, 4, 1, 1,  1), 0, 0, 0},
     {0, 0, 0, 0, job1(0, 0, 0, 0, 0, 0, 0), 0, 0, 0}};
 
-static size_t build_wgrad_table(int cus, WgradTable& t, bool legacy, int mult = 0) {
+static size_t build_wgrad_table(int cus, WgradTable& t, bool legacy, int mult = 0, int fixed = 0) {
   const WgradPlan* plan = legacy ? kWgradPlan : kWgradPlanTr;
   int n = 0;
   double cost[16], total = 0;
@@ -2238,6 +2268,7 @@
     const WgradPlan& p = plan[i];
     int share = (int)(budget * cost[i] / total + 0.5);
     if (share < 8) share = 8;
+    if (fixed > 0) share = fixed;
     t.qx[i] = p.qx; t.KSx[i] = p.KSx; t.qd[i] = p.qd; t.KSd[i] = p.KSd; t.job[i] = p.job;
     t.qx2[i] = p.qx2; t.qd2[i] = p.qd2; t.KSd2[i] = p.KSd2;
     t.wg0[i] = wg; wg += share;
@@ -2286,12 +2317,43 @@
   }
 };
 
+static int launch_wgrad_reduce(const WgradTable& tab, const float* workspace, float* grads, const float* out_scale, hipStream_t st) {
+  int max_elems = 0, max_cols = 0;
+  for (int j = 0; j < tab.n; ++j) {
+    max_elems = tab.job[j].KT * tab.job[j].NT * 1024 > max_elems ? tab.job[j].KT * tab.job[j].NT * 1024 : max_elems;
+    max_cols = tab.job[j].NT * 32 > max_cols ? tab.job[j].NT * 32 : max_cols;
+  }
+  const int elem_blocks = (max_elems / 4 + 255) / 256;
+  hipLaunchKernelGGL(wgrad_reduce_kernel, dim3(elem_blocks + (max_cols + 255) / 256, tab.n), dim3(256), 0, st, workspace, tab, grads, out_scale, elem_blocks);
+  RNERF_CHECK_LAUNCH();
+  return RNERF_OK;
+}
+
+#ifdef RNERF_EXPERIMENTS
+extern "C" int rnerf_test_wgrad_reduce(int32_t wgs_per_job, const float* workspace, float* grads, int64_t* layout, void* stream) {
+  RNERF_CHECK_ARG(layout && wgs_per_job >= 0 && wgs_per_job <= 64, "rnerf_test_wgrad_reduce: bad arguments");
+  WgradTable own;
+  size_t floats = wgrad_tables().partial_floats;
+  if (wgs_per_job > 0) floats = build_wgrad_table(device_cus(), own, false, 0, wgs_per_job);
+  const WgradTable& tab = wgs_per_job > 0 ? own : wgrad_tables().tr;
+  layout[0] = tab.n; layout[1] = (int64_t)floats;
+  for (int j = 0; j < tab.n; ++j) {
+    int64_t* l = layout + 2 + 5 * j;
+    l[0] = tab.job[j].KT; l[1] = tab.job[j].NT; l[2] = tab.wg0[j + 1] - tab.wg0[j]; l[3] = tab.poff[j]; l[4] = tab.pboff[j];
+  }
+  if (!workspace) return RNERF_OK;
+  RNERF_CHECK_ARG(grads && ((uintptr_t)workspace & 15) == 0, "rnerf_test_wgrad_reduce: grads is null or the workspace is not 16-byte aligned");
+  return launch_wgrad_reduce(tab, workspace, grads, nullptr, (hipStream_t)stream);
+}
+#endif
+
 extern "C" int rnerf_nerfmlp_wgrad(int fwd_precision, int backward, const void* save, const void* dy, int64_t rows, float* grads, void* workspace,
                                    void* stream) {
   RNERF_CHECK_ARG(save && dy && grads && workspace, "rnerf_nerfmlp_wgrad: null pointer");
   RNERF_CHECK_ARG(train_combo_ok(fwd_precision, backward), "rnerf_nerfmlp_wgrad: forward precision must be f16x3 (f16 with a single-plane backward mode; bf16x3 with backward bf16)");
   RNERF_CHECK_ARG(bwd_ok(backward), "rnerf_nerfmlp_wgrad: unknown backward mode %d", backward);
   RNERF_CHECK_ARG(rows >= 1, "rnerf_nerfmlp_wgrad: rows must be >= 1");
+  RNERF_CHECK_ARG(((uintptr_t)workspace & 15) == 0, "rnerf_nerfmlp_wgrad: workspace must be 16-byte aligned");
   const WgradTables& w = wgrad_tables();
   static DeviceOnce ready;
   if (ready.need()) {
@@ -2323,10 +2385,7 @@
   } else {
     out_scale = WgradTrHost<F16Planes<2>>::launch(tab, st, save, dy, R, workspace, trace);
   }
-  int max_elems = 0;
-  for (int j = 0; j < tab.n; ++j) max_elems = tab.job[j].KT * tab.job[j].NT * 1024 > max_elems ? tab.job[j].KT * tab.job[j].NT * 1024 : max_elems;
-  hipLaunchKernelGGL(wgrad_reduce_kernel, dim3((max_elems + 255) / 256, tab.n), dim3(256), 0, st, (const float*)workspace, tab, grads, out_scale);
-  RNERF_CHECK_LAUNCH();
+  RNERF_TRY_(launch_wgrad_reduce(tab, (const float*)workspace, grads, out_scale, st));
   if (trace && backward != RNERF_BWD_BF16) {
     const int n_wg = tab.wg0[tab.n];
     std::vector<long long> h(2 * (size_t)n_wg);
diff --git a/samplenerfro_amd/csrc/pipeline.hip b/samplenerfro_amd/csrc/pipeline.hip
--- a/samplenerfro_amd/csrc/pipeline.hip
+++ b/samplenerfro_amd/csrc/pipeline.hip
@@ -507,7 +507,7 @@
 }
 
 static int mark_point(hipStream_t first, hipEvent_t* out);
-static int wait_point(hipStream_t then, hipEvent_t e);
+static int wait_point(hipStream_t then, hipEvent_t e, bool keep = false);
 
 extern "C" int rnerf_train_forward_backward(const rnerf_model* m, const rnerf_train_cfg* c, const float* theta, const float* origins, const float* viewdirs,
                                             const float* pixels, const float* env_dirs, int32_t B, const uint32_t* keys4, const int32_t* jitter_override,
@@ -543,7 +543,8 @@
 
   void* aux = c->aux_stream;
   bool pre_zeroed = false;
-  struct Mark { hipEvent_t e = nullptr; ~Mark() { if (e) pool_put(e); } } fine_packed;
+  struct Mark { hipEvent_t e = nullptr; ~Mark() { if (e) pool_put(e); } };
+  Mark fine_packed;
   if (aux) {
     RNERF_TRY(rnerf_fork(stream, aux));
     void* streams[2] = {t.packed_c, t.packed_f};
@@ -574,9 +575,9 @@
       RNERF_TRY(mark_point((hipStream_t)aux, &fine_packed.e));
     }
     RNERF_CHECK_HIP(hipMemsetAsync(grads, 0, (size_t)(n_theta + 8) * sizeof(float), (hipStream_t)aux));
+    RNERF_TRY(rnerf_theta_sumsq(theta, n_theta, stats8, aux));
     RNERF_TRY(rnerf_nerfmlp_pack_bwd(th_c, bwd, t.packed_bwd, aux));
     if (Nf > 0) RNERF_TRY(rnerf_nerfmlp_pack_bwd(th_f, bwd, t.packed_bwd_f, aux));
-    RNERF_TRY(rnerf_theta_sumsq(theta, n_theta, stats8, aux));
   } else {
     RNERF_TRY(rnerf_nerfmlp_pack(th_c, prec, t.packed_c, stream));
   }
@@ -603,9 +604,10 @@
   const double mse_scale = 2.0 / (3.0 * B);
   const double env_on = c->annealed_alpha > 0 ? 1.0 : 0.0;
   if (!aux) RNERF_CHECK_HIP(hipMemsetAsync(grads, 0, (size_t)(n_theta + 8) * sizeof(float), st));
-  auto march_next = [&]() -> int {
+  auto march_next = [&](hipEvent_t after = nullptr) -> int {
     RNERF_CHECK_ARG(next->origins && next->viewdirs && next->path_pd && next->path_dr && next->side_stream, "rnerf_train_forward_backward: incomplete rnerf_prefetch");
-    RNERF_TRY(rnerf_fork(stream, next->side_stream));
+    if (after) RNERF_TRY(wait_point((hipStream_t)next->side_stream, after,  true));
+    else RNERF_TRY(rnerf_fork(stream, next->side_stream));
     return rnerf_march(m->table, &m->grid, next->origins, next->viewdirs, B, m->near, m->far, N, next->path_pd, next->path_dr, nullptr, nullptr,
                        next->side_stream);
   };
@@ -642,10 +644,19 @@
   if (!aux) RNERF_TRY(rnerf_nerfmlp_pack_bwd(th_c, bwd, t.packed_bwd, stream));
   if (!split_levels)
     RNERF_TRY(nerfmlp_dgrad_impl(t.packed_bwd, t.packed_c, prec, bwd, t.save_c, t.d_raw, (int64_t)Nc * B, t.dy, !(pre_zeroed && Nf == 0), true, st));
-  if (next && Nf == 0) RNERF_TRY(march_next());
   const bool tail_on_aux = aux && !split_levels;
+  Mark after_dgrad;
+  if (next && Nf == 0) {
+    if (tail_on_aux) {
+      RNERF_TRY(mark_point(st, &after_dgrad.e));
+      RNERF_TRY(march_next(after_dgrad.e));
+    } else {
+      RNERF_TRY(march_next());
+    }
+  }
   void* tail = tail_on_aux ? aux : stream;
-  if (tail_on_aux) RNERF_TRY(rnerf_fork(stream, aux));
+  if (after_dgrad.e) { hipEvent_t e = after_dgrad.e; after_dgrad.e = nullptr; RNERF_TRY(wait_point((hipStream_t)aux, e)); }
+  else if (tail_on_aux) RNERF_TRY(rnerf_fork(stream, aux));
   if (!split_levels && !tail_on_aux) RNERF_TRY(rnerf_nerfmlp_wgrad(prec, bwd, t.save_c, t.dy, (int64_t)Nc * B, g_c, t.wgrad_ws, stream));
   if (!tail_on_aux && c->grads_stream) RNERF_TRY(rnerf_fork(stream, c->grads_stream));
   if (!split_levels) {
@@ -791,11 +802,12 @@
   *out = e;
   return RNERF_OK;
 }
-static int wait_point(hipStream_t then, hipEvent_t e) {
+static int wait_point(hipStream_t then, hipEvent_t e, bool keep) {
   hipStreamCaptureStatus cs = hipStreamCaptureStatusNone;
   hipError_t err = hipStreamIsCapturing(then, &cs);
   if (err == hipSuccess) err = hipStreamWaitEvent(then, e, 0);
-  if (err != hipSuccess) { (void)hipEventDestroy(e); set_error("stream ordering failed: %s", hipGetErrorString(err)); return RNERF_ERR_HIP; }
+  if (err != hipSuccess) { if (!keep) (void)hipEventDestroy(e); set_error("stream ordering failed: %s", hipGetErrorString(err)); return RNERF_ERR_HIP; }
+  if (keep) return RNERF_OK;
   if (cs == hipStreamCaptureStatusNone) pool_put(e);
   else tl_capture_events.push_back(e);
   return RNERF_OK;
diff --git a/samplenerfro_amd/train.py b/samplenerfro_amd/train.py
--- a/samplenerfro_amd/train.py
+++ b/samplenerfro_amd/train.py
@@ -360,7 +360,14 @@
             state._lag_host[slot:slot + 1].copy_(state.adam_scratch[3:4], non_blocking=True)
         ev = torch.cuda.Event(); ev.record()
         replay = dict(kw, next_rays=None, path=None)
-        state._lag_pending.append((ev, slot, rng, _clone_batch(batch), flags, replay, ctx))
+        if _takes_whole_path(model, flags, kw):
+            cur, aux = torch.cuda.current_stream(), model.tail_stream()
+            with torch.cuda.stream(aux):
+                kept = _clone_batch(batch)
+            cur.wait_stream(aux)
+        else:
+            kept = _clone_batch(batch)
+        state._lag_pending.append((ev, slot, rng, kept, flags, replay, ctx))
         state._model_ref = weakref.ref(model)
         while len(state._lag_pending) > _RANGE_RETRY_LAG:
             pend = state._lag_pending.pop(0)
@@ -469,6 +476,12 @@
         _settle_lagged(model, state, state._lag_pending.pop(0))
 
 
+def _takes_whole_path(model: NerfModel, flags, kw) -> bool:
+    noisy = getattr(model, "noise_std", None) is not None and bool(flags.randomized)
+    return (flags.stage.startswith("radiance") and kw.get("taps") is None and kw.get("forward_taps") is None
+            and bool(getattr(model, "whole_path", False)) and not noisy)
+
+
 def _train_step_once(model: NerfModel, rng, state: TrainState, batch: Dict[str, Any], flags=None, *, jitter=None, u_fine=None,
                      taps: Optional[dict] = None, path=None, next_rays: Optional[Rays] = None, forward_taps: Optional[dict] = None,
                      noise_c=None, noise_f=None, _guard: bool = False):
@@ -482,8 +495,7 @@
         raise ValueError("stage all*: build the model with the same stage (the march must evaluate so3_mlp)")
     if flags.beta_weight > 0 or flags.sparsity_weight > 0:
         pass
-    noisy = getattr(model, "noise_std", None) is not None and bool(flags.randomized)
-    if not all_stage and taps is None and forward_taps is None and getattr(model, "whole_path", False) and not noisy:
+    if _takes_whole_path(model, flags, dict(taps=taps, forward_taps=forward_taps)):
         return _train_step_whole(model, rng, state, batch, flags, jitter, u_fine, path, next_rays)
     rng, key_0, key_1 = prng.split(np.asarray(rng, np.uint32), 3)
     annealed = float(np.asarray(batch["annealed_alpha"]).reshape(-1)[0])
```

New measurement: 666,500, median of 6. About the same (+0.6%).
